# samuel-vitorino/sopro

Measured on AMD Instinct MI355X. Metric: audio_seconds_per_second, higher is better.
Workload: dtype f32; 1 GPU; Sopro-135M synthesize, 32 utterances x 200 frames per GPU (BASELINE configs[1]), S=64 text tokens, 32 distinct 150-frame reference voice(s) per batch prepared outside the timed region, top_p=0.9 T=1.05 anti_loop (reference defaults), synthetic weights with EOS suppressed; batch_per_gpu=32, frames=200, voices_per_batch=32, parallelism=replicas x1 (utterance sharding, no collective), lanes_per_gpu=4

## Files before the change

include/sopro_hip.h:

```cpp
#ifndef SOPRO_HIP_H
#define SOPRO_HIP_H

#include <stdint.h>

#ifdef __cplusplus
extern "C" {
#endif

#define SOPRO_ABI_VERSION 43

const char* sopro_last_error(void);
int sopro_abi_version(void);
int sopro_build_flags(void);
int sopro_set_lds_floor(int bytes);
int sopro_set_host_wait(int blocking);
int sopro_device_info(int device, int* out4);

int sopro_capture_begin(void* stream);
int sopro_capture_end(void* stream, void** graph_exec_out);
int sopro_graph_launch(void* graph_exec, void* stream);
int sopro_graph_launch_n(void* graph_exec, void* stream, int32_t n);
int sopro_graph_destroy(void* graph_exec);
int sopro_stream_create_cu_range(int first_cu, int n_cus, void** stream_out);
int sopro_stream_create_cu_mask(const uint32_t* mask, int32_t words, void** stream_out);
// ... 14 lines not shown
  float* C; int64_t ldc; int64_t c_seg_stride;
  const float* R; int64_t ldr; int64_t r_seg_stride;
  const float* scale;
  const float* pro_vec;
  long long* dbg;
  int32_t M, N, K, rows_per_seg;
  int32_t prologue, epilogue;
} sopro_gemm_args;
int sopro_gemm_f32(const sopro_gemm_args* args, void* stream);
int sopro_gemm_set_tile_override(int cfg);

typedef struct sopro_gemm_split_ext {
  int32_t a_format;
  int32_t c_mode;
  float* C2; int64_t ldc2; int64_t c2_seg_stride;
  int32_t rms_norm; float rms_eps;
  int32_t ksplit;
  int32_t n_tickets;
  float* ws; int64_t ws_bytes;
  int32_t* tickets;
  int32_t group_m;
  float acc_scale;
  int32_t* range_events;
  const float* rope_cos; const float* rope_sin;
  int32_t rope_cols, rope_dh, rope_pos0, rope_rows_per_seg;
  const float* ln_stats;
  float* ln_stats_out;
} sopro_gemm_split_ext;
int sopro_gemm_bf16x3(const sopro_gemm_args* a, const void* packed_w, const sopro_gemm_split_ext* ext, void* stream);
int64_t sopro_packed_w_rows_bytes(int32_t N, int32_t K);
int sopro_pack_w_rows_bf16(const float* W, int64_t ldw, int32_t N, int32_t K, void* packed, void* stream);
int sopro_gemm_8p_takes(const sopro_gemm_args* a, const sopro_gemm_split_ext* ext);
int sopro_gemm_bf16x3_8p(const sopro_gemm_args* a, const void* w_rows, const sopro_gemm_split_ext* ext, void* stream);
int sopro_gemm_bf16x6(const sopro_gemm_args* a, const void* packed_w, const sopro_gemm_split_ext* ext, void* stream);
int sopro_gemm_bf16x1(const sopro_gemm_args* a, const void* packed_w, const sopro_gemm_split_ext* ext, void* stream);
int sopro_pack_w_bf16(const float* W, int64_t ldw, int32_t N, int32_t K, int32_t pieces, void* packed, void* stream);
int sopro_pack_w_f16x2(const float* W, int64_t ldw, int32_t N, int32_t K, float wscale, void* packed, void* stream);
float sopro_f16x3_a_scale(void);
int sopro_gemm_f16x3(const sopro_gemm_args* a, const void* packed_w, const sopro_gemm_split_ext* ext, void* stream);
int64_t sopro_packed_w_bytes(int32_t N, int32_t K, int32_t pieces);
int sopro_gemm_bf16_set_tile_override(int cfg);
int sopro_gemm_set_group_m(int g);
int sopro_gemm_auto_ksplit(int32_t M, int32_t N, int32_t K, int32_t pieces, int32_t f16, int32_t epilogue, int64_t ws_bytes, int32_t n_tickets);

typedef struct sopro_skinny_args {
  const float* X; int64_t ldx;
  const float* W; int64_t ldw;
  const float* bias;
  float* Y; int64_t ldy;
  const float* R; int64_t ldr;
  const float* scale;
  float* ring;
  const float* dw_w;
  const float* dw_b;
  const int32_t* step;
  const float* Xp; int64_t xp_stride;
  int64_t y_part_stride;
  long long* dbg;
  float eps;
  int32_t B, N, K, epilogue;
  int32_t ring_len, ring_bcap, dil, ksize;
  int32_t np, ksplit, rms_norm;
  int32_t w_layout;
  const float* aux_W; const float* aux_bias; const float* aux_R; float* aux_Y;
  int64_t aux_ldy, aux_ldr, aux_y_part_stride;
  int32_t aux_tiles, aux_flags;
  int32_t ring_format;
  int32_t mt, nt;
} sopro_skinny_args;
int sopro_skinny_f32(const sopro_skinny_args* args, void* stream);
int sopro_pack_skinny_w(const float* W, int64_t ldw, int32_t N, int32_t K, int32_t glu, float* out, void* stream);
int64_t sopro_skinny_packed_floats(int32_t N, int32_t K, int32_t glu);
int sopro_pack_skinny_w_bf16(const float* W, int64_t ldw, int32_t N, int32_t K, int32_t glu, void* out, void* stream);

int sopro_fill2d_u32(void* p, int64_t pitch, int32_t rows, int32_t width, uint32_t value, void* stream);
int sopro_copy2d_u32(void* dst, int64_t dpitch, const void* src, int64_t spitch, int32_t rows, int32_t width, void* stream);
int sopro_nar_seed_i32(int32_t* tokens, int32_t Q, const int32_t* cb0, int64_t cb0_bstride, int32_t B, int32_t T, int32_t vmax, void* stream);
int sopro_cvt_f32_bf16(const float* src, void* dst, int64_t n, void* stream);
int sopro_cvt_bf16_f32(const void* src, float* dst, int64_t n, void* stream);
enum { SOPRO_NORM_RMS = 0, SOPRO_NORM_LN = 1 };
int sopro_norm_f32(const float* x, int64_t ldx, int64_t x_seg_stride , float* out, int64_t ldo, const float* w, const float* b,
                   const float* mul, const float* add, int32_t rows, int32_t rows_per_seg, int32_t C,
                   float eps, int32_t kind, void* stream);
int sopro_row_stats_f32(const float* x, int64_t ldx, int64_t x_seg_stride , int32_t rows, int32_t rows_per_seg, int32_t C,
                        float* stats, void* stream);
int sopro_rms_match_f32(const float* a, const float* x, float* out, int32_t rows, int32_t C, void* stream);
int sopro_tanh_affine_f32(const float* in, float* out, float c0, float c1, int64_t n, void* stream);
int sopro_add_pos_f32(const float* rowvec, const float* table, float* out, int32_t B, int32_t T, int32_t C,
                      int32_t pos0, void* stream);
int sopro_masked_mean_f32(const float* x, const int32_t* lens, float* out, int32_t B, int32_t T, int32_t C,
                          void* stream);

int sopro_stats_pool_f32(const float* h, const float* logit, const int32_t* lens, float* out, int32_t B, int32_t T,
                         int32_t C, void* stream);
int sopro_l2norm_f32(const float* x, float* out, int32_t rows, int32_t C, float eps, void* stream);

int sopro_dwconv_f32(const float* x, const float* w, const float* bias, const float* res, float* out,
                     const int32_t* lens, int32_t B, int32_t T, int32_t C, int32_t ksize, int32_t dil,
                     int32_t left, int32_t mode, void* stream);

int sopro_codebook_sum_f32(const int32_t* tok, int32_t ldt, const int32_t* col, const int32_t* off, const float* wq,
                           int32_t nq, const float* table, int64_t table_rows, const float* base, float alpha,
                           float beta, float* out, int64_t ldo, int64_t o_seg_stride, int32_t rows,
                           int32_t rows_per_seg, int32_t D, void* stream);
int sopro_text_embed_f32(const int32_t* ids, const int32_t* lens, const float* table, int64_t table_rows,
                         const float* pe, float* out, int32_t B, int32_t T, int32_t C, void* stream);
int sopro_argmax_rows_f32(const float* x, int64_t ldx, int32_t* out, int64_t ldo, int32_t inner, int32_t rows, int32_t N,
                          void* stream);
int sopro_argmax_partials_i32(const float* partials, int64_t ldp, int32_t* out, int64_t ldo, int32_t heads, int32_t per_head, int32_t V,
                              int32_t rows, void* stream);

int sopro_fir1_f32(const float* x, int64_t x_seg_stride, int32_t n_in, const float* w, const float* bias, float* out,
                   int64_t ldo, int64_t o_seg_stride, int32_t B, int32_t n_out, int32_t C, int32_t K, int32_t stride,
                   int32_t left, void* stream);
int sopro_rvq_assign_f32(const float* scores, int64_t lds, int32_t V, const float* table, float* res, int64_t ldr,
                         int32_t D, int32_t* codes, int64_t ldc, int32_t rows, void* stream);

typedef struct sopro_attn_args {
  const float* Q; int64_t ldq; int64_t q_bstride;
  const float* K; int64_t ldk; int64_t k_bstride;
  const float* V; int64_t ldv; int64_t v_bstride;
  float* O; int64_t ldo; int64_t o_bstride;
  const int32_t* klens;
  int32_t B, H, dh, Tq, Tk;
  int32_t causal, q_pos0, k_pos0, window;
  float scale;
  const int32_t* kv_index;
} sopro_attn_args;
int sopro_attention_f32(const sopro_attn_args* args, void* stream);
int sopro_attention_split_bf16(const sopro_attn_args* args, int32_t passes, void* stream);
int sopro_attn_decode_f32(const sopro_attn_args* args, void* stream);
typedef struct sopro_xattn_args {
  const float* X; int64_t ldx;
  const float* Xp; int64_t xp_stride;
  const float* norm_w;
  const float* Kp; const float* Vp;
  const int32_t* klens;
  float* Y; int64_t y_part_stride;
  float eps, gate, scale;
  int32_t np, B, H, D, S_cap;
  const float* Qp; int64_t qp_stride;
  int32_t nqp, k_unfolded;
  int32_t kv_format;
} sopro_xattn_args;
int sopro_xattn_step_f32(const sopro_xattn_args* args, void* stream);

int sopro_rope_f32(float* x, int64_t ldx, const float* cos_t, const float* sin_t, int32_t rows,
                   int32_t rows_per_seg, int32_t pos0, int32_t H, int32_t dh, void* stream);

int sopro_upsample2_f32(const float* x, const float* w, float* y, int64_t y_seg_stride, int32_t B, int32_t T,
                        int32_t C, void* stream);
int sopro_final_conv_f32(const float* h, int64_t h_seg_stride, const float* w, float bias, float* wav,
                         int64_t wav_seg_stride, int32_t B, int32_t T, void* stream);

int sopro_seanet_tail_f32(const float* h, int64_t h_seg_stride, const float* w1, const float* b1, const float* w2,
                          const float* b2, const float* wf, float bf, float* wav, int64_t wav_seg_stride, int32_t B,
                          int32_t T, void* stream);
int sopro_seanet_tail_p_f32(const float* h, int64_t h_seg_stride, const float* w1, const float* b1, const float* w2,
                            const float* b2, const float* wf, float bf, float* wav, int64_t wav_seg_stride, int32_t B,
                            int32_t T, int32_t passes, void* stream);
int sopro_seanet_res128_f32(const float* h, int64_t h_seg_stride, const float* w1, const float* b1, const float* w2, const float* b2,
                            float* out, int64_t out_seg_stride, int32_t B, int32_t T, void* stream);
int sopro_seanet_res128_p_f32(const float* h, int64_t h_seg_stride, const float* w1, const float* b1, const float* w2, const float* b2,
                              float* out, int64_t out_seg_stride, int32_t B, int32_t T, int32_t passes , void* stream);
int sopro_seanet_res_set_tiles(int tiles);
int sopro_seanet_up128_f32(const float* x, int64_t x_seg_stride, const float* w, const float* bias, float* out,
// ... 325 lines not shown
```

sopro_amd/csrc/common.h:

```cpp
#pragma once
#ifdef SOPRO_DEV_SWITCHES
#define SOPRO_DEV_ENV(name) getenv(name)
#else
#define SOPRO_DEV_ENV(name) (static_cast<const char*>(nullptr))
#endif
#include <hip/hip_runtime.h>
#include <stdint.h>
#include <stdio.h>
#include <string.h>

#include "../../include/sopro_hip.h"

typedef float f32x4 __attribute__((ext_vector_type(4)));
typedef float f32x16 __attribute__((ext_vector_type(16)));

void sopro_set_error(const char* fmt, ...);
extern int g_sopro_lds_floor;

#define SOPRO_CHECK_ARG(cond, msg)                                  \
  do {                                                              \
    if (!(cond)) {                                                  \
      sopro_set_error("%s: bad argument: %s", __func__, msg);       \
      return -2;                                                    \
    }                                                               \
  } while (0)

#define SOPRO_HIP(call)                                                                   \
  do {                                                                                    \
    hipError_t e_ = (call);                                                               \
    if (e_ != hipSuccess) {                                                               \
      sopro_set_error("%s: %s failed: %s", __func__, #call, hipGetErrorString(e_));       \
      return -1;                                                                          \
    }                                                                                     \
  } while (0)

#define SOPRO_LAUNCH_CHECK()                                                              \
  do {                                                                                    \
    hipError_t e_ = hipGetLastError();                                                    \
    if (e_ != hipSuccess) {                                                               \
      sopro_set_error("%s: kernel launch failed: %s", __func__, hipGetErrorString(e_));   \
      return -1;                                                                          \
    }                                                                                     \
    return 0;                                                                             \
  } while (0)

static inline bool aligned16(const void* p) { return (reinterpret_cast<uintptr_t>(p) & 15u) == 0; }

#define SOPRO_SET_MAX_LDS_ONCE(kern, bytes)                                                                              \
  do {                                                                                                                   \
    static unsigned char done_[64] = {};                                                                                 \
    int dev_ = 0;                                                                                                        \
    SOPRO_HIP(hipGetDevice(&dev_));                                                                                      \
    if (!done_[dev_ & 63]) {                                                                                             \
      SOPRO_HIP(hipFuncSetAttribute(reinterpret_cast<const void*>(kern), hipFuncAttributeMaxDynamicSharedMemorySize, (int)(bytes))); \
      done_[dev_ & 63] = 1;                                                                                              \
    }                                                                                                                    \
  } while (0)

__device__ __forceinline__ float gelu_erf(float v) { return v * 0.5f * (1.0f + erff(v * 0.70710678118654752440f)); }
__device__ __forceinline__ float gelu_fast(float v) {
  const float x = fabsf(v) * 0.70710678118654752440f;
  const float t = __builtin_amdgcn_rcpf(fmaf(0.3275911f, x, 1.0f));
  float p = fmaf(1.061405429f, t, -1.453152027f);
  p = fmaf(p, t, 1.421413741f);
  p = fmaf(p, t, -0.284496736f);
  p = fmaf(p, t, 0.254829592f);
  p *= t;
  const float e = __builtin_amdgcn_exp2f(x * x * -1.44269504088896340736f);
  const float y = fmaf(-p, e, 1.0f);
  const float h = 0.5f * v;
  return fmaf(h, copysignf(y, v), h);
}
__device__ __forceinline__ float sigmoidf_(float v) { return 1.0f / (1.0f + expf(-v)); }
__device__ __forceinline__ float sigmoid_fast(float v) { return __builtin_amdgcn_rcpf(1.0f + __builtin_amdgcn_exp2f(-1.44269504088896340736f * v)); }
__device__ __forceinline__ float eluf_(float v) { return __builtin_amdgcn_fmed3f(v, __expf(v) - 1.0f, 0.0f); }

typedef __bf16 bf16x2_t __attribute__((ext_vector_type(2)));
typedef float f32x2_t __attribute__((ext_vector_type(2)));
__device__ __forceinline__ void split2_bf16(float x, float y, unsigned& hi, unsigned& lo) {
  const f32x2_t v = {x, y};
  const bf16x2_t h = __builtin_convertvector(v, bf16x2_t);
  hi = *reinterpret_cast<const unsigned*>(&h);
  const f32x2_t r = {x - __uint_as_float(hi << 16), y - __uint_as_float(hi & 0xffff0000u)};
  const bf16x2_t l = __builtin_convertvector(r, bf16x2_t);
  lo = *reinterpret_cast<const unsigned*>(&l);
}

#ifndef SOPRO_NT_BULK
#define SOPRO_NT_BULK 1
#endif
__device__ __forceinline__ bool bulk_nt(bool big) { return SOPRO_NT_BULK == 1 || (SOPRO_NT_BULK == 2 && big); }
typedef unsigned u32x4_t __attribute__((ext_vector_type(4)));
typedef unsigned u32x2_t __attribute__((ext_vector_type(2)));
__device__ __forceinline__ void bulk_store4(float* p, const float4& v, bool big) {
  if (bulk_nt(big)) __builtin_nontemporal_store((f32x4){v.x, v.y, v.z, v.w}, reinterpret_cast<f32x4*>(p));
  else *reinterpret_cast<float4*>(p) = v;
}
__device__ __forceinline__ void bulk_store1(float* p, float v, bool big) {
  if (bulk_nt(big)) __builtin_nontemporal_store(v, p);
  else *p = v;
}
__device__ __forceinline__ void bulk_store_u2(void* p, const uint2& v, bool big) {
  if (bulk_nt(big)) __builtin_nontemporal_store((u32x2_t){v.x, v.y}, reinterpret_cast<u32x2_t*>(p));
  else *reinterpret_cast<uint2*>(p) = v;
}
__device__ __forceinline__ void bulk_store_u1(void* p, unsigned v, bool big) {
  if (bulk_nt(big)) __builtin_nontemporal_store(v, reinterpret_cast<unsigned*>(p));
  else *reinterpret_cast<unsigned*>(p) = v;
}
__device__ __forceinline__ uint4 bulk_load16(const void* p, bool big) {
  if (bulk_nt(big)) {
    const u32x4_t v = __builtin_nontemporal_load(reinterpret_cast<const u32x4_t*>(p));
    return make_uint4(v.x, v.y, v.z, v.w);
  }
  return *reinterpret_cast<const uint4*>(p);
}
constexpr int64_t SOPRO_BIG_BYTES = (int64_t)64 << 20;

__device__ __forceinline__ int xcd_contiguous(int b, int n) {
  const int per = n >> 3, rem = n & 7;
  const int x = b & 7, i = b >> 3;
  return x * per + min(x, rem) + i;
}

__device__ __forceinline__ float wave_sum(float v) {
#pragma unroll
  for (int o = 32; o > 0; o >>= 1) v += __shfl_xor(v, o, 64);
  return v;
}
__device__ __forceinline__ float wave_max(float v) {
#pragma unroll
  for (int o = 32; o > 0; o >>= 1) v = fmaxf(v, __shfl_xor(v, o, 64));
  return v;
}

__device__ __forceinline__ void wave_lds_sync() {
  __builtin_amdgcn_fence(__ATOMIC_RELEASE, "wavefront");
  __builtin_amdgcn_wave_barrier();
  __builtin_amdgcn_fence(__ATOMIC_ACQUIRE, "wavefront");
}

struct sopro_prof_scope {
  void* rec;
  hipStream_t s;
  sopro_prof_scope(const char* family, double flops, hipStream_t s);
  ~sopro_prof_scope();
  sopro_prof_scope(const sopro_prof_scope&) = delete;
  sopro_prof_scope& operator=(const sopro_prof_scope&) = delete;
};
```

sopro_amd/csrc/elementwise.hip:

```cpp
#include "common.h"

namespace {

constexpr int NORM_MAX_PER_LANE = 16;

__global__ __launch_bounds__(256) void norm_kernel(const float* __restrict__ x, int64_t ldx, int64_t x_seg_stride, float* __restrict__ out,
                                                   int64_t ldo, const float* __restrict__ w, const float* __restrict__ b,
                                                   const float* __restrict__ mul, const float* __restrict__ add, int rows,
                                                   int rows_per_seg, int C, float eps, int kind) {
  const int lane = threadIdx.x & 63;
  const int row = blockIdx.x * 4 + (threadIdx.x >> 6);
  if (row >= rows) return;
  const int seg = row / rows_per_seg;
  const float* xr = x + (int64_t)seg * x_seg_stride + (int64_t)(row - seg * rows_per_seg) * ldx;
  float v[NORM_MAX_PER_LANE];
  const int per = (C + 63) / 64;
  float s = 0.f;
#pragma unroll
  for (int j = 0; j < NORM_MAX_PER_LANE; ++j) {
    const int c = lane + j * 64;
    v[j] = (j < per && c < C) ? xr[c] : 0.f;
    s += v[j];
  }
  float mean = 0.f, var;
  if (kind == SOPRO_NORM_LN) {
    mean = wave_sum(s) / (float)C;
    float q = 0.f;
#pragma unroll
    for (int j = 0; j < NORM_MAX_PER_LANE; ++j) {
      const int c = lane + j * 64;
      const float d = (j < per && c < C) ? v[j] - mean : 0.f;
      q += d * d;
    }
    var = wave_sum(q) / (float)C;
  } else {
    float q = 0.f;
#pragma unroll
    for (int j = 0; j < NORM_MAX_PER_LANE; ++j) q += v[j] * v[j];
    var = wave_sum(q) / (float)C;
  }
  const float rstd = rsqrtf(var + eps);
  const float* mr = mul ? mul + (int64_t)seg * C : nullptr;
  const float* ar = add ? add + (int64_t)seg * C : nullptr;
  float* orow = out + (int64_t)row * ldo;
#pragma unroll
  for (int j = 0; j < NORM_MAX_PER_LANE; ++j) {
    const int c = lane + j * 64;
    if (j < per && c < C) {
      float y = ((v[j] - mean) * rstd) * w[c];
      if (b) y += b[c];
      if (mr) y *= mr[c];
      if (ar) y += ar[c];
      orow[c] = y;
    }
  }
}

__global__ __launch_bounds__(256) void rms_match_kernel(const float* __restrict__ a, const float* __restrict__ x,
                                                        float* __restrict__ out, int rows, int C) {
  const int lane = threadIdx.x & 63;
  const int row = blockIdx.x * 4 + (threadIdx.x >> 6);
  if (row >= rows) return;
  const float* ar = a + (int64_t)row * C;
  const float* xr = x + (int64_t)row * C;
  float sa = 0.f, sx = 0.f;
  for (int c = lane; c < C; c += 64) {
    sa += ar[c] * ar[c];
    sx += xr[c] * xr[c];
  }
  sa = wave_sum(sa);
  sx = wave_sum(sx);
  const float ra = sqrtf(sa / (float)C + 1e-6f), rx = sqrtf(sx / (float)C + 1e-6f);
  const float sc = fminf(fmaxf(rx / ra, 0.f), 10.f);
  for (int c = lane; c < C; c += 64) out[(int64_t)row * C + c] = ar[c] * sc;
}

__global__ void tanh_affine_kernel(const float* __restrict__ in, float* __restrict__ out, float c0, float c1, int64_t n) {
  const int64_t i = (int64_t)blockIdx.x * blockDim.x + threadIdx.x;
  if (i < n) out[i] = c0 + c1 * tanhf(in[i]);
}

__global__ void add_pos_kernel(const float* __restrict__ rowvec, const float* __restrict__ table, float* __restrict__ out,
                               int B, int T, int C, int pos0) {
  const int64_t i = (int64_t)blockIdx.x * blockDim.x + threadIdx.x;
  const int64_t n = (int64_t)B * T * C;
  if (i >= n) return;
  const int c = (int)(i % C);
  const int64_t bt = i / C;
  const int t = (int)(bt % T), b = (int)(bt / T);
  out[i] = rowvec[(int64_t)b * C + c] + table[(int64_t)(pos0 + t) * C + c];
}

__global__ void masked_mean_kernel(const float* __restrict__ x, const int* __restrict__ lens, float* __restrict__ out,
                                   int B, int T, int C) {
  const int b = blockIdx.y;
  const int c = blockIdx.x * blockDim.x + threadIdx.x;
  if (c >= C) return;
  const int len = lens ? min(lens[b], T) : T;
  float s = 0.f;
  for (int t = 0; t < len; ++t) s += x[((int64_t)b * T + t) * C + c];
  out[(int64_t)b * C + c] = s / ((float)len + 1e-6f);
}

__global__ __launch_bounds__(256) void dwconv_kernel(const float* __restrict__ x, const float* __restrict__ w,
                                                     const float* __restrict__ bias, const float* __restrict__ res,
                                                     float* __restrict__ out, const int* __restrict__ lens, int B, int T,
                                                     int C, int ksize, int dil, int left, int mode) {
  const int c4n = C >> 2;
  const int64_t i = (int64_t)blockIdx.x * blockDim.x + threadIdx.x;
  if (i >= (int64_t)B * T * c4n) return;
  const int c4 = (int)(i % c4n);
  const int64_t bt = i / c4n;
  const int t = (int)(bt % T), b = (int)(bt / T);
  const int len = lens ? min(lens[b], T) : T;
  float4 acc = make_float4(0.f, 0.f, 0.f, 0.f);
  for (int j = 0; j < ksize; ++j) {
    const int ts = t - left + j * dil;
    if (ts < 0 || ts >= len) continue;
    const float4 xv = *reinterpret_cast<const float4*>(x + ((int64_t)b * T + ts) * C + c4 * 4);
    const float4 wv = *reinterpret_cast<const float4*>(w + (int64_t)j * C + c4 * 4);
    acc.x += xv.x * wv.x; acc.y += xv.y * wv.y; acc.z += xv.z * wv.z; acc.w += xv.w * wv.w;
  }
  if (bias) {
    const float4 bv = *reinterpret_cast<const float4*>(bias + c4 * 4);
    acc.x += bv.x; acc.y += bv.y; acc.z += bv.z; acc.w += bv.w;
  }
  const int64_t o = ((int64_t)b * T + t) * C + c4 * 4;
  if (mode == 1) {
    const float4 rv = *reinterpret_cast<const float4*>(res + o);
    acc.x += rv.x; acc.y += rv.y; acc.z += rv.z; acc.w += rv.w;
  } else if (mode == 2) {
    acc.x = gelu_erf(acc.x); acc.y = gelu_erf(acc.y); acc.z = gelu_erf(acc.z); acc.w = gelu_erf(acc.w);
  }
  *reinterpret_cast<float4*>(out + o) = acc;
}

template <int KS>
// ... 311 lines not shown
  if (row >= rows) return;
  float s = 0.f;
  for (int c = lane; c < C; c += 64) s += x[(int64_t)row * C + c] * x[(int64_t)row * C + c];
  s = wave_sum(s);
  const float d = fmaxf(sqrtf(s), eps);
  for (int c = lane; c < C; c += 64) out[(int64_t)row * C + c] = x[(int64_t)row * C + c] / d;
}

inline unsigned nblk(int64_t n, int bs) { return (unsigned)((n + bs - 1) / bs); }


__global__ __launch_bounds__(256) void fill2d_kernel(unsigned* __restrict__ p, int64_t pitch, int rows, int width, unsigned v) {
  const int64_t i = (int64_t)blockIdx.x * blockDim.x + threadIdx.x;
  if (i >= (int64_t)rows * width) return;
  p[(i / width) * pitch + (i % width)] = v;
}
__global__ __launch_bounds__(256) void copy2d_kernel(unsigned* __restrict__ d, int64_t dpitch, const unsigned* __restrict__ s, int64_t spitch, int rows,
                                                     int width) {
  const int64_t i = (int64_t)blockIdx.x * blockDim.x + threadIdx.x;
  if (i >= (int64_t)rows * width) return;
  d[(i / width) * dpitch + (i % width)] = s[(i / width) * spitch + (i % width)];
}

__global__ __launch_bounds__(256) void nar_seed_kernel(int* __restrict__ tokens, int Q, const int* __restrict__ cb0, int64_t bstride, int B, int T, int vmax) {
  const int64_t i = (int64_t)blockIdx.x * blockDim.x + threadIdx.x;
  if (i >= (int64_t)B * T) return;
  const int b = (int)(i / T), t = (int)(i - (int64_t)b * T);
  tokens[i * Q] = min(max(cb0[(int64_t)b * bstride + t], 0), vmax);
}

__global__ __launch_bounds__(256) void cvt_f32_bf16_kernel(const float* __restrict__ src, uint2* __restrict__ dst, int64_t n4) {
  const int64_t i = (int64_t)blockIdx.x * blockDim.x + threadIdx.x;
  if (i >= n4) return;
  const float4 v = reinterpret_cast<const float4*>(src)[i];
  unsigned a, b, lo;
  split2_bf16(v.x, v.y, a, lo);
  split2_bf16(v.z, v.w, b, lo);
  dst[i] = make_uint2(a, b);
}
__global__ __launch_bounds__(256) void cvt_bf16_f32_kernel(const uint2* __restrict__ src, float* __restrict__ dst, int64_t n4) {
  const int64_t i = (int64_t)blockIdx.x * blockDim.x + threadIdx.x;
  if (i >= n4) return;
  const uint2 v = src[i];
  reinterpret_cast<float4*>(dst)[i] = make_float4(__uint_as_float(v.x << 16), __uint_as_float(v.x & 0xffff0000u), __uint_as_float(v.y << 16),
                                                  __uint_as_float(v.y & 0xffff0000u));
}

__global__ __launch_bounds__(256) void row_stats_kernel(const float* __restrict__ x, int64_t ldx, int64_t seg_stride, int rows, int rps, int C,
                                                        float* __restrict__ stats) {
  const int per_row = C >> 2;
  const int64_t i = (int64_t)blockIdx.x * blockDim.x + threadIdx.x;
  const int64_t r = i / per_row;
  if (r >= rows) return;
  const int c4 = (int)(i - r * per_row);
  const int64_t seg = r / rps, rr = r - seg * rps;
  const float4 v = *reinterpret_cast<const float4*>(x + seg * seg_stride + rr * ldx + c4 * 4);
  float s = (v.x + v.y) + (v.z + v.w);
  s += __shfl_xor(s, 1, 64); s += __shfl_xor(s, 2, 64); s += __shfl_xor(s, 4, 64); s += __shfl_xor(s, 8, 64);
  const float mu = s * (1.0f / 64.0f);
  const float dx = v.x - mu, dy = v.y - mu, dz = v.z - mu, dw = v.w - mu;
  float q = (dx * dx + dy * dy) + (dz * dz + dw * dw);
  q += __shfl_xor(q, 1, 64); q += __shfl_xor(q, 2, 64); q += __shfl_xor(q, 4, 64); q += __shfl_xor(q, 8, 64);
  if ((c4 & 15) == 0) *reinterpret_cast<float2*>(stats + (r * (C >> 6) + (c4 >> 4)) * 2) = make_float2(mu, q);
}

}

extern "C" {

int sopro_row_stats_f32(const float* x, int64_t ldx, int64_t x_seg_stride, int32_t rows, int32_t rows_per_seg, int32_t C, float* stats, void* stream) {
  SOPRO_CHECK_ARG(x && stats && rows > 0 && rows_per_seg > 0 && C > 0 && (C & 63) == 0, "x, stats non-NULL; rows > 0; C a multiple of 64");
  SOPRO_CHECK_ARG(aligned16(x) && (ldx & 3) == 0 && (x_seg_stride & 3) == 0 && (reinterpret_cast<uintptr_t>(stats) & 7u) == 0, "16-byte aligned rows, 8-byte aligned stats");
  hipLaunchKernelGGL(row_stats_kernel, dim3(nblk((int64_t)rows * (C >> 2), 256)), dim3(256), 0, (hipStream_t)stream, x, ldx,
                     x_seg_stride ? x_seg_stride : (int64_t)rows_per_seg * ldx, rows, rows_per_seg, C, stats);
  SOPRO_LAUNCH_CHECK();
}

int sopro_norm_f32(const float* x, int64_t ldx, int64_t x_seg_stride, float* out, int64_t ldo, const float* w, const float* b,
                   const float* mul, const float* add, int32_t rows, int32_t rows_per_seg, int32_t C, float eps,
                   int32_t kind, void* stream) {
  SOPRO_CHECK_ARG(x && out && w, "x, out, w must be non-NULL");
  SOPRO_CHECK_ARG(rows > 0 && C > 0 && C <= 64 * NORM_MAX_PER_LANE && rows_per_seg > 0, "rows > 0, 0 < C <= 1024");
  SOPRO_CHECK_ARG(kind == SOPRO_NORM_RMS || kind == SOPRO_NORM_LN, "unknown norm kind");
  hipLaunchKernelGGL(norm_kernel, dim3(nblk(rows, 4)), dim3(256), 0, (hipStream_t)stream, x, ldx,
                     x_seg_stride ? x_seg_stride : (int64_t)rows_per_seg * ldx, out, ldo, w, b, mul, add, rows, rows_per_seg, C, eps, kind);
  SOPRO_LAUNCH_CHECK();
}

int sopro_rms_match_f32(const float* a, const float* x, float* out, int32_t rows, int32_t C, void* stream) {
  SOPRO_CHECK_ARG(a && x && out && rows > 0 && C > 0, "bad pointers or sizes");
  hipLaunchKernelGGL(rms_match_kernel, dim3(nblk(rows, 4)), dim3(256), 0, (hipStream_t)stream, a, x, out, rows, C);
  SOPRO_LAUNCH_CHECK();
}

int sopro_tanh_affine_f32(const float* in, float* out, float c0, float c1, int64_t n, void* stream) {
  SOPRO_CHECK_ARG(in && out && n > 0, "bad pointers or sizes");
  hipLaunchKernelGGL(tanh_affine_kernel, dim3(nblk(n, 256)), dim3(256), 0, (hipStream_t)stream, in, out, c0, c1, n);
  SOPRO_LAUNCH_CHECK();
}

int sopro_add_pos_f32(const float* rowvec, const float* table, float* out, int32_t B, int32_t T, int32_t C, int32_t pos0,
                      void* stream) {
  SOPRO_CHECK_ARG(rowvec && table && out && B > 0 && T > 0 && C > 0 && pos0 >= 0, "bad pointers or sizes");
  hipLaunchKernelGGL(add_pos_kernel, dim3(nblk((int64_t)B * T * C, 256)), dim3(256), 0, (hipStream_t)stream, rowvec, table,
                     out, B, T, C, pos0);
  SOPRO_LAUNCH_CHECK();
}

int sopro_masked_mean_f32(const float* x, const int32_t* lens, float* out, int32_t B, int32_t T, int32_t C, void* stream) {
  SOPRO_CHECK_ARG(x && out && B > 0 && T > 0 && C > 0, "bad pointers or sizes");
  hipLaunchKernelGGL(masked_mean_kernel, dim3(nblk(C, 128), B), dim3(128), 0, (hipStream_t)stream, x, lens, out, B, T, C);
  SOPRO_LAUNCH_CHECK();
}

int sopro_dwconv_f32(const float* x, const float* w, const float* bias, const float* res, float* out, const int32_t* lens,
                     int32_t B, int32_t T, int32_t C, int32_t ksize, int32_t dil, int32_t left, int32_t mode, void* stream) {
  SOPRO_CHECK_ARG(x && w && out && B > 0 && T > 0 && C > 0 && (C & 3) == 0, "bad pointers or sizes (C % 4 == 0)");
  SOPRO_CHECK_ARG(ksize >= 1 && dil >= 1 && left >= 0 && mode >= 0 && mode <= 2, "bad conv geometry or mode");
  SOPRO_CHECK_ARG(mode != 1 || res, "mode 1 needs res");
  SOPRO_CHECK_ARG(aligned16(x) && aligned16(w) && aligned16(out), "pointers must be 16-byte aligned");
  SOPRO_CHECK_ARG((!bias || aligned16(bias)) && (!res || aligned16(res)), "bias / res must be 16-byte aligned");
  static const bool comb_off = SOPRO_DEV_ENV("SOPRO_DWCONV_COMB") != nullptr && SOPRO_DEV_ENV("SOPRO_DWCONV_COMB")[0] == '0';
  if (!comb_off && (ksize == 11 || ksize == 7) && (int64_t)B * T >= 1024 && T >= 8 * dil) {
    const int per_r = ((T + dil - 1) / dil + 7) / 8;
    const dim3 grid(nblk((int64_t)B * dil * per_r * (C / 4), 256));
    if (ksize == 11)
      hipLaunchKernelGGL(dwconv_comb_kernel<11>, grid, dim3(256), 0, (hipStream_t)stream, x, w, bias, res, out, lens, B, T, C, dil, left, mode, per_r);
    else
      hipLaunchKernelGGL(dwconv_comb_kernel<7>, grid, dim3(256), 0, (hipStream_t)stream, x, w, bias, res, out, lens, B, T, C, dil, left, mode, per_r);
    SOPRO_LAUNCH_CHECK();
  }
  hipLaunchKernelGGL(dwconv_kernel, dim3(nblk((int64_t)B * T * (C / 4), 256)), dim3(256), 0, (hipStream_t)stream, x, w, bias,
                     res, out, lens, B, T, C, ksize, dil, left, mode);
  SOPRO_LAUNCH_CHECK();
}

int sopro_codebook_sum_f32(const int32_t* tok, int32_t ldt, const int32_t* col, const int32_t* off, const float* wq,
                           int32_t nq, const float* table, int64_t table_rows, const float* base, float alpha, float beta,
                           float* out, int64_t ldo, int64_t o_seg_stride, int32_t rows, int32_t rows_per_seg, int32_t D,
                           void* stream) {
  SOPRO_CHECK_ARG(tok && col && off && wq && table && out, "NULL pointer");
  SOPRO_CHECK_ARG(rows > 0 && rows_per_seg > 0 && nq > 0 && D > 0 && (D & 3) == 0 && table_rows > 0, "bad sizes (D % 4 == 0)");
  SOPRO_CHECK_ARG(aligned16(table) && aligned16(out) && (ldo & 3) == 0 && (o_seg_stride & 3) == 0, "alignment");
  hipLaunchKernelGGL(codebook_sum_kernel, dim3(nblk((int64_t)rows * (D / 4), 256)), dim3(256), 0, (hipStream_t)stream, tok,
                     ldt, col, off, wq, nq, table, table_rows, base, alpha, beta, out, ldo, o_seg_stride, rows, rows_per_seg, D);
  SOPRO_LAUNCH_CHECK();
}

int sopro_text_embed_f32(const int32_t* ids, const int32_t* lens, const float* table, int64_t table_rows, const float* pe,
                         float* out, int32_t B, int32_t T, int32_t C, void* stream) {
  SOPRO_CHECK_ARG(ids && table && pe && out && B > 0 && T > 0 && C > 0 && (C & 3) == 0, "bad pointers or sizes");
  hipLaunchKernelGGL(text_embed_kernel, dim3(nblk((int64_t)B * T * (C / 4), 256)), dim3(256), 0, (hipStream_t)stream, ids, lens,
                     table, table_rows, pe, out, B, T, C);
  SOPRO_LAUNCH_CHECK();
}

int sopro_argmax_rows_f32(const float* x, int64_t ldx, int32_t* out, int64_t ldo, int32_t inner, int32_t rows, int32_t N,
                          void* stream) {
  SOPRO_CHECK_ARG(x && out && rows > 0 && N > 0 && inner > 0, "bad pointers or sizes");
  hipLaunchKernelGGL(argmax_rows_kernel, dim3(nblk(rows, 4)), dim3(256), 0, (hipStream_t)stream, x, ldx, out, ldo, inner, rows, N);
  SOPRO_LAUNCH_CHECK();
}

int sopro_fir1_f32(const float* x, int64_t x_seg_stride, int32_t n_in, const float* w, const float* bias, float* out, int64_t ldo,
                   int64_t o_seg_stride, int32_t B, int32_t n_out, int32_t C, int32_t K, int32_t stride, int32_t left, void* stream) {
  SOPRO_CHECK_ARG(x && w && out, "NULL pointer");
  SOPRO_CHECK_ARG(B > 0 && B <= 65535 && n_in > 0 && n_out > 0 && C > 0 && K > 0 && stride > 0 && left >= 0 && ldo >= C, "bad sizes");
  hipLaunchKernelGGL(fir1_kernel, dim3(nblk((int64_t)n_out * C, 256), B), dim3(256), 0, (hipStream_t)stream, x, x_seg_stride, n_in, w,
// ... 154 lines not shown
```

sopro_amd/csrc/gemm_bf16s.hip:

```cpp
#include "common.h"
#include "gemm_epilogue.h"
#include "gemm_host.h"

namespace {

constexpr int BK = 32;


typedef __bf16 bf16x8 __attribute__((ext_vector_type(8)));
typedef _Float16 f16x8 __attribute__((ext_vector_type(8)));
typedef _Float16 f16x2_t __attribute__((ext_vector_type(2)));

__device__ __forceinline__ bf16x8 as_frag(const uint4& v) { return *reinterpret_cast<const bf16x8*>(&v); }
__device__ __forceinline__ f16x8 as_frag16(const uint4& v) { return *reinterpret_cast<const f16x8*>(&v); }

constexpr float A16_SCALE = 8.0f;

template <int NPL, bool F16 = false>
__device__ __forceinline__ void split_pair(float x, float y, unsigned (&pc)[NPL]) {
#pragma unroll
  for (int p = 0; p < NPL; ++p) {
    const f32x2_t v = {x, y};
    if constexpr (F16) {
      const f16x2_t h = __builtin_convertvector(v, f16x2_t);
      pc[p] = *reinterpret_cast<const unsigned*>(&h);
      x -= (float)h[0];
      y -= (float)h[1];
    } else {
      const bf16x2_t h = __builtin_convertvector(v, bf16x2_t);
      pc[p] = *reinterpret_cast<const unsigned*>(&h);
      x -= __uint_as_float(pc[p] << 16);
      y -= __uint_as_float(pc[p] & 0xffff0000u);
    }
  }
}

template <int NPL, int WM, int WN, int TM, int TN, int EPI, int AMODE, int OUT, bool SK, bool F16 = false>
__global__ __launch_bounds__(WM* WN * 64) void gemm_bf16s_kernel(const sopro_gemm_args g, const uint4* __restrict__ Wp,
                                                                 int ksubs, const sopro_gemm_split_ext ext) {
  constexpr int AROW = NPL * 64 + 16;
  constexpr bool FOLD = F16;
  constexpr int NT = WM * WN * 64;
  constexpr int BM = WM * TM * 32;
  constexpr int BN = WN * TN * 32;
  constexpr int A_F4 = BM * 8 / NT;
  constexpr int RSTEP = NT / 8;
  extern __shared__ float4 smem4[];
  unsigned char* As = reinterpret_cast<unsigned char*>(smem4);

  const int tid = threadIdx.x, lane = tid & 63, wave = tid >> 6;
  const int wm = wave / WN, wn = wave % WN;
  const int ntn = (g.N + BN - 1) / BN;
  const int bid = xcd_contiguous((int)blockIdx.x, (int)gridDim.x);
  int mt = bid / ntn, nt = bid % ntn;
  if (ext.group_m > 1) {
    const int ntm_all = (g.M + BM - 1) / BM;
    const int per = ext.group_m * ntn;
    const int grp = bid / per, rem = bid - grp * per;
    const int first = grp * ext.group_m;
    const int gsz = min(ntm_all - first, ext.group_m);
    mt = first + rem % gsz;
    nt = rem / gsz;
  }
  const int m0 = mt * BM, n0 = nt * BN;
  const int lrow = tid >> 3, lc4 = tid & 7;
  const int rps = g.rows_per_seg;
  long long* dbg = g.dbg ? g.dbg + (int64_t)blockIdx.x * 8 : nullptr;
  if (dbg && tid == 0) dbg[0] = clock64();

  static_assert(AMODE != 5 || NPL == 1, "bf16 rows are a one-pass (bf16 mode) operand form");
  constexpr int AES = AMODE == 5 ? 2 : 4;
  const char* ap[A_F4];
#pragma unroll
  for (int i = 0; i < A_F4; ++i) {
    const int m = min(m0 + lrow + i * RSTEP, g.M - 1);
    const int seg = m / rps;
    const int r = m - seg * rps;
    ap[i] = reinterpret_cast<const char*>(g.A) + ((int64_t)seg * g.a_seg_stride + (int64_t)r * g.lda) * AES;
  }
  const int ntiles = (g.N + 31) >> 5;
  const uint4* bp[TN];
#pragma unroll
  for (int j = 0; j < TN; ++j) {
    const int t = min((n0 >> 5) + wn * TN + j, ntiles - 1);
    bp[j] = Wp + ((int64_t)t * ksubs * NPL) * 64 + lane;
  }
  int boff[TN];
#pragma unroll
  for (int j = 0; j < TN; ++j) {
    const int t = min((n0 >> 5) + wn * TN + j, ntiles - 1);
    boff[j] = (t * ksubs * NPL) * 64 + lane;
  }
  float biasv[TN];
#pragma unroll
  for (int j = 0; j < TN; ++j) {
    const int n = n0 + (wn * TN + j) * 32 + (lane & 31);
    biasv[j] = (g.bias && n < g.N) ? g.bias[n] : 0.f;
  }

  float4 raA[A_F4], raB[A_F4];
  float ssq[A_F4];
  float rsc[A_F4];
  float a16max = 0.f;
#pragma unroll
  for (int i = 0; i < A_F4; ++i) { ssq[i] = 0.f; rsc[i] = A16_SCALE; }
  float sapin[A_F4];
#pragma unroll
  for (int i = 0; i < A_F4; ++i) sapin[i] = A16_SCALE;
  float lmu[A_F4], lrs[A_F4];
  float4 pvA = make_float4(0.f, 0.f, 0.f, 0.f), pvB = pvA;
  const int KT = (g.K + BK - 1) / BK;
  const int klast = g.K - 4;

  auto gload = [&](int kt, float4 (&ra)[A_F4], float4& pv) {
    const int k = min(kt * BK + lc4 * 4, klast);
    if constexpr (AMODE == 5) {
#pragma unroll
      for (int i = 0; i < A_F4; ++i) {
        const uint2 v = *reinterpret_cast<const uint2*>(ap[i] + (int64_t)k * 2);
        ra[i].x = __uint_as_float(v.x);
        ra[i].y = __uint_as_float(v.y);
      }
    } else {
#pragma unroll
      for (int i = 0; i < A_F4; ++i) ra[i] = *reinterpret_cast<const float4*>(ap[i] + (int64_t)k * 4);
    }
    if (AMODE == 3) pv = *reinterpret_cast<const float4*>(g.pro_vec + k);
  };
  auto bload = [&](int kt, uint4 (&rb)[TN][2][NPL]) {
#pragma unroll
    for (int j = 0; j < TN; ++j)
#pragma unroll
      for (int s = 0; s < 2; ++s)
#pragma unroll
        for (int p = 0; p < NPL; ++p) rb[j][s][p] = bp[j][((int64_t)(kt * 2 + s) * NPL + p) * 64];
  };
  auto lstore_piece = [&](int buf, float4 (&ra)[A_F4], const float4& pv, int i, bool fresh, bool first) {
    if constexpr (FOLD) {
      if constexpr (AMODE == 4) asm volatile("" : "+v"(rsc[i]), "+v"(ssq[i]));
      else asm volatile("" : "+v"(sapin[i]));
    }
    if constexpr (AMODE == 5) {
      unsigned char* a = As + buf * BM * AROW + lrow * AROW + lc4 * 8;
      *reinterpret_cast<uint2*>(a + i * RSTEP * AROW) = make_uint2(__float_as_uint(ra[i].x), __float_as_uint(ra[i].y));
    } else if constexpr (AMODE == 2) {
      unsigned char* a = As + buf * BM * AROW + lrow * AROW + lc4 * 16;
      *reinterpret_cast<f32x4*>(a + i * RSTEP * AROW) = (f32x4){ra[i].x, ra[i].y, ra[i].z, ra[i].w};
    } else {
      if constexpr (AMODE == 1) {
        ra[i].x = eluf_(ra[i].x); ra[i].y = eluf_(ra[i].y); ra[i].z = eluf_(ra[i].z); ra[i].w = eluf_(ra[i].w);
      } else if constexpr (AMODE == 3) {
        ra[i].x += pv.x; ra[i].y += pv.y; ra[i].z += pv.z; ra[i].w += pv.w;
      } else if constexpr (AMODE == 6) {
        const f32x2_t r2 = {lrs[i], lrs[i]}, n2 = {lmu[i], lmu[i]};
        const f32x2_t lo2 = (f32x2_t){ra[i].x, ra[i].y} * r2 + n2, hi2 = (f32x2_t){ra[i].z, ra[i].w} * r2 + n2;
        ra[i].x = lo2[0]; ra[i].y = lo2[1]; ra[i].z = hi2[0]; ra[i].w = hi2[1];
      }
      if constexpr (AMODE == 4) {
        if (fresh) ssq[i] = fmaf(ra[i].x, ra[i].x, fmaf(ra[i].y, ra[i].y, fmaf(ra[i].z, ra[i].z, fmaf(ra[i].w, ra[i].w, ssq[i]))));
      }
      unsigned char* a = As + buf * BM * AROW + lrow * AROW + lc4 * 8;
      {
        unsigned c0[NPL], c1[NPL];
        if constexpr (F16) {
          const float F16MAX = 65504.0f;
          if constexpr (AMODE == 4) {
            if (first) {
              float mx = fmaxf(fmaxf(fabsf(ra[i].x), fabsf(ra[i].y)), fmaxf(fabsf(ra[i].z), fabsf(ra[i].w)));
              mx = fmaxf(mx, __shfl_xor(mx, 1, 64));
              mx = fmaxf(mx, __shfl_xor(mx, 2, 64));
              mx = fmaxf(mx, __shfl_xor(mx, 4, 64));
              const int ex = (int)((__float_as_uint(mx) >> 23) & 255u);
              rsc[i] = (ex == 0 || ex == 255) ? A16_SCALE : __uint_as_float((unsigned)min(max(261 - ex, 2), 252) << 23);
            }
          }
          const float sa = AMODE == 4 ? rsc[i] : sapin[i];
          const float vx = ra[i].x * sa, vy = ra[i].y * sa, vz = ra[i].z * sa, vw = ra[i].w * sa;
          a16max = fmaxf(a16max, fmaxf(fmaxf(fabsf(vx), fabsf(vy)), fmaxf(fabsf(vz), fabsf(vw))));
          split_pair<NPL, true>(__builtin_amdgcn_fmed3f(vx, -F16MAX, F16MAX), __builtin_amdgcn_fmed3f(vy, -F16MAX, F16MAX), c0);
          split_pair<NPL, true>(__builtin_amdgcn_fmed3f(vz, -F16MAX, F16MAX), __builtin_amdgcn_fmed3f(vw, -F16MAX, F16MAX), c1);
        } else {
          split_pair<NPL>(ra[i].x, ra[i].y, c0);
          split_pair<NPL>(ra[i].z, ra[i].w, c1);
        }
#pragma unroll
        for (int p = 0; p < NPL; ++p) *reinterpret_cast<uint2*>(a + i * RSTEP * AROW + p * 64) = make_uint2(c0[p], c1[p]);
      }
    }
  };
  auto lstore = [&](int buf, float4 (&ra)[A_F4], const float4& pv, bool fresh = true, bool first = false) {
#pragma unroll
    for (int i = 0; i < A_F4; ++i) lstore_piece(buf, ra, pv, i, fresh, first);
  };

  f32x16 acc[TM][TN];
#pragma unroll
  for (int i = 0; i < TM; ++i)
#pragma unroll
    for (int j = 0; j < TN; ++j)
#pragma unroll
      for (int r = 0; r < 16; ++r) acc[i][j][r] = 0.f;

  const int frow = lane & 31, fg = lane >> 5;
  constexpr int NPAIR = NPL == 1 ? 1 : (NPL == 2 ? 3 : 6);
  constexpr int PA[6] = {NPL == 1 ? 0 : (NPL == 2 ? 1 : 2), 0, NPL == 2 ? 0 : 1, 1, 0, 0};
  constexpr int PB[6] = {0, NPL == 2 ? 1 : 2, NPL == 2 ? 0 : 1, 0, 1, 0};
  auto compute = [&](int buf, const uint4 (&rb)[TN][2][NPL]) {
    const unsigned char* a = As + buf * BM * AROW + (wm * TM * 32 + frow) * AROW + fg * 16;
#pragma unroll
    for (int s = 0; s < 2; ++s) {
      uint4 af[TM][NPL];
#pragma unroll
      for (int i = 0; i < TM; ++i)
#pragma unroll
        for (int p = 0; p < NPL; ++p) af[i][p] = *reinterpret_cast<const uint4*>(a + i * 32 * AROW + p * 64 + s * 32);
#pragma unroll
      for (int q = 0; q < NPAIR; ++q)
#pragma unroll
        for (int i = 0; i < TM; ++i)
#pragma unroll
          for (int j = 0; j < TN; ++j)
            if constexpr (F16)
              acc[i][j] = __builtin_amdgcn_mfma_f32_32x32x16_f16(as_frag16(af[i][PA[q]]), as_frag16(rb[j][s][PB[q]]), acc[i][j], 0, 0, 0);
// ... 41 lines not shown
          for (int j = 0; j < TN; ++j) {
            if constexpr (F16)
              acc[i][j] = __builtin_amdgcn_mfma_f32_32x32x16_f16(as_frag16(af[i][PA[q]]), as_frag16(rb[j][s][PB[q]]), acc[i][j], 0, 0, 0);
            else
              acc[i][j] = __builtin_amdgcn_mfma_f32_32x32x16_bf16(as_frag(af[i][PA[q]]), as_frag(rb[j][s][PB[q]]), acc[i][j], 0, 0, 0);
            ++m;
            if constexpr (FOLD) {
#pragma unroll
              for (int i = 0; i < A_F4; ++i)
                if (m == NM / 2 + i * (NM / 2) / A_F4) {
                  __builtin_amdgcn_sched_barrier(0x104);
                  lstore_piece(buf ^ 1, rs, pvs, i, fresh_s, false);
                }
            }
            if (m % STRIDE == 0 && nl < NL) {
              if constexpr (NPL == 1) {
                __builtin_amdgcn_sched_barrier(0);
                issue(nl++);
                __builtin_amdgcn_sched_barrier(0);
              } else {
                __builtin_amdgcn_sched_barrier(0x786);
                issue(nl++);
                __builtin_amdgcn_sched_barrier(0x786);
              }
            }
          }
    }
#pragma unroll
    for (int n = 0; n < NL; ++n)
      if (n >= nl) issue(n);
  };

  const int KS = SK ? ext.ksplit : 1;
  const int per = (KT + KS - 1) / KS;
  const int kt0 = (int)blockIdx.y * per;
  const int nkt = max(0, min(KT, kt0 + per) - kt0);
  const int ktl = max(kt0, kt0 + nkt - 1);

  uint4 rb0[TN][2][NPL], rb1[TN][2][NPL];
  constexpr bool DEEP = true;
  gload(min(kt0, KT - 1), raA, pvA);
  bload(min(kt0, KT - 1), rb0);
  if (DEEP) gload(min(min(kt0 + 1, ktl), KT - 1), raB, pvB);
  if constexpr (AMODE == 6) {
    const int P = g.K >> 6;
#pragma unroll
    for (int i = 0; i < A_F4; ++i) {
      const float2* st = reinterpret_cast<const float2*>(ext.ln_stats) + (int64_t)min(m0 + lrow + i * RSTEP, g.M - 1) * P;
      float sm = 0.f;
      for (int p = lc4; p < P; p += 8) sm += st[p].x;
      sm += __shfl_xor(sm, 1, 64); sm += __shfl_xor(sm, 2, 64); sm += __shfl_xor(sm, 4, 64);
      const float mean = sm / (float)P;
      float m2 = 0.f;
      for (int p = lc4; p < P; p += 8) {
        const float2 v = st[p];
        const float d = v.x - mean;
        m2 += fmaf(64.0f * d, d, v.y);
      }
      m2 += __shfl_xor(m2, 1, 64); m2 += __shfl_xor(m2, 2, 64); m2 += __shfl_xor(m2, 4, 64);
      lrs[i] = rsqrtf(m2 / (float)g.K + ext.rms_eps);
      lmu[i] = -mean * lrs[i];
    }
  }
  lstore(0, raA, pvA, true, true);
  __syncthreads();
  if (dbg && tid == 0) dbg[1] = clock64();
  {
    int it = 0;
    for (; it + 1 < nkt; it += 2) {
      const int k1 = min(kt0 + it + 1, ktl), k2 = min(kt0 + it + 2, ktl), k3 = min(kt0 + it + 3, ktl);
      compute_spread(0, rb0, k2, raA, pvA, k1, rb1, raB, pvB, true);
      if constexpr (!FOLD) lstore(1, raB, pvB, true);
      __syncthreads();
      compute_spread(1, rb1, k3, raB, pvB, k2, rb0, raA, pvA, it + 2 < nkt);
      if constexpr (!FOLD) lstore(0, raA, pvA, it + 2 < nkt);
      __syncthreads();
    }
    if (it < nkt) {
      compute(0, rb0);
      __syncthreads();
    }
  }
  if (dbg && tid == 0) dbg[2] = clock64();
  if constexpr (SK) {
    constexpr int PER_THREAD = TM * TN * 16;
    const int tile = bid, ntile = gridDim.x;
    float* mine = ext.ws + ((int64_t)((int64_t)blockIdx.y * ntile + tile) * NT + tid) * PER_THREAD;
#pragma unroll
    for (int i = 0; i < TM; ++i)
#pragma unroll
      for (int j = 0; j < TN; ++j)
#pragma unroll
        for (int r = 0; r < 16; r += 4)
          *reinterpret_cast<float4*>(mine + (i * TN + j) * 16 + r) = make_float4(acc[i][j][r], acc[i][j][r + 1], acc[i][j][r + 2], acc[i][j][r + 3]);
    __syncthreads();
    int* flag = reinterpret_cast<int*>(smem4);
    if (tid == 0) {
      __atomic_thread_fence(__ATOMIC_RELEASE);
      const int old = __hip_atomic_fetch_add(ext.tickets + tile, 1, __ATOMIC_ACQ_REL, __HIP_MEMORY_SCOPE_AGENT);
      *flag = old;
      if (old == KS - 1) __hip_atomic_store(ext.tickets + tile, 0, __ATOMIC_RELAXED, __HIP_MEMORY_SCOPE_AGENT);
    }
    __syncthreads();
    if (*flag != KS - 1) return;
    __atomic_thread_fence(__ATOMIC_ACQUIRE);
    __syncthreads();
#pragma unroll
    for (int i = 0; i < TM; ++i)
#pragma unroll
      for (int j = 0; j < TN; ++j)
#pragma unroll
        for (int r = 0; r < 16; ++r) acc[i][j][r] = 0.f;
    const int64_t sl_stride = (int64_t)ntile * NT * PER_THREAD;
    const float* part0 = ext.ws + ((int64_t)tile * NT + tid) * PER_THREAD;
    for (int s0 = 0; s0 < KS; s0 += 16) {
#pragma unroll
      for (int i = 0; i < TM; ++i)
#pragma unroll
        for (int j = 0; j < TN; ++j)
#pragma unroll
          for (int r = 0; r < 16; r += 4) {
            f32x4 v[16];
#pragma unroll
            for (int u = 0; u < 16; ++u) {
              const int sl = min(s0 + u, KS - 1);
              v[u] = __builtin_nontemporal_load(reinterpret_cast<const f32x4*>(part0 + sl * sl_stride + (i * TN + j) * 16 + r));
            }
#pragma unroll
            for (int u = 0; u < 16; ++u) {
              if (s0 + u < KS) {
                acc[i][j][r] += v[u][0]; acc[i][j][r + 1] += v[u][1]; acc[i][j][r + 2] += v[u][2]; acc[i][j][r + 3] += v[u][3];
              }
            }
          }
    }
  }
  float cscale = 1.0f;
  if constexpr (F16) {
    cscale = AMODE == 4 ? ext.acc_scale * A16_SCALE : ext.acc_scale;
    if (ext.range_events && !(a16max <= 65504.0f)) atomicAdd(ext.range_events, 1);
  }
  const float* rs = nullptr;
  if constexpr (AMODE == 4) {
    float* rsl = reinterpret_cast<float*>(smem4) + BM * (BN + 4);
#pragma unroll
    for (int i = 0; i < A_F4; ++i) {
      float v = ssq[i];
      v += __shfl_xor(v, 1, 64);
      v += __shfl_xor(v, 2, 64);
      v += __shfl_xor(v, 4, 64);
      float r = rsqrtf(v / (float)g.K + ext.rms_eps);
      if constexpr (F16) r *= __uint_as_float(0x7f000000u - __float_as_uint(rsc[i])) * cscale;
      if (lc4 == 0) rsl[lrow + i * RSTEP] = r;
    }
    __syncthreads();
    rs = rsl;
  }
  gemm_store_tile<WM, WN, TM, TN, EPI, OUT>(g, reinterpret_cast<float*>(smem4), acc, biasv, m0, n0, &ext, rs, cscale);
  if (dbg && tid == 0) dbg[3] = clock64();
}

template <int NPL, bool F16 = false>
__global__ __launch_bounds__(256) void pack_w_kernel(const float* __restrict__ W, int64_t ldw, int N, int K, uint4* __restrict__ out,
                                                     int ksubs, int64_t total, float wscale = 1.0f) {
  const int64_t i = (int64_t)blockIdx.x * blockDim.x + threadIdx.x;
  if (i >= total) return;
  const int lane = (int)(i & 63);
  const int64_t pk = i >> 6;
  const int p = (int)(pk % NPL);
  const int64_t tk = pk / NPL;
  const int ks = (int)(tk % ksubs);
  const int t = (int)(tk / ksubs);
  const int n = t * 32 + (lane & 31);
  const int k0 = ks * 16 + (lane >> 5) * 8;
  unsigned w[4];
#pragma unroll
  for (int e = 0; e < 4; ++e) {
    const int k = k0 + 2 * e;
    const float x = (n < N && k < K) ? W[(int64_t)n * ldw + k] : 0.f;
    const float y = (n < N && k + 1 < K) ? W[(int64_t)n * ldw + k + 1] : 0.f;
    unsigned pc[NPL];
    if constexpr (F16) split_pair<NPL, true>(x * wscale, y * wscale, pc);
    else split_pair<NPL>(x, y, pc);
    w[e] = pc[p];
  }
  out[i] = make_uint4(w[0], w[1], w[2], w[3]);
}

template <int NPL, int WM, int WN, int TM, int TN, int EPI, int AMODE, int OUT, bool F16 = false>
int launch_one(const sopro_gemm_args& g, const uint4* wp, int ksubs, const sopro_gemm_split_ext& ext, hipStream_t s) {
  constexpr int BM = WM * TM * 32, BN = WN * TN * 32;
  constexpr size_t lds_main = (size_t)2 * BM * (NPL * 64 + 16), lds_epi = (size_t)BM * (BN + 4 + (AMODE == 4 ? 1 : 0)) * sizeof(float);
  constexpr size_t lds = lds_main > lds_epi ? lds_main : lds_epi;
  const int ks = ext.ksplit > 1 ? ext.ksplit : 1;
  auto kern = ks > 1 ? gemm_bf16s_kernel<NPL, WM, WN, TM, TN, EPI, AMODE, OUT, true, F16> : gemm_bf16s_kernel<NPL, WM, WN, TM, TN, EPI, AMODE, OUT, false, F16>;
  constexpr size_t lds_cap = lds > (size_t)96 * 1024 ? lds : (size_t)96 * 1024;
  if (ks > 1) SOPRO_SET_MAX_LDS_ONCE(kern, lds_cap);
  else SOPRO_SET_MAX_LDS_ONCE(kern, lds_cap);
  const size_t lds_req = lds > (size_t)g_sopro_lds_floor ? lds : (size_t)g_sopro_lds_floor;
  const int ntm = (g.M + BM - 1) / BM, ntn = (g.N + BN - 1) / BN;
  if (ks > 1) {
    const int64_t need = (int64_t)ks * ntm * ntn * BM * BN * (int64_t)sizeof(float);
    if (!ext.ws || !ext.tickets || ext.ws_bytes < need || ext.n_tickets < ntm * ntn) {
      sopro_set_error("split-K needs a %lld-byte workspace and %d tickets (got %lld, %d)", (long long)need, ntm * ntn,
                      (long long)ext.ws_bytes, ext.n_tickets);
      return -2;
    }
  }
  hipLaunchKernelGGL(kern, dim3(ntm * ntn, ks), dim3(WM * WN * 64), lds_req, s, g, wp, ksubs, ext);
  SOPRO_LAUNCH_CHECK();
}

inline int amode_of(const sopro_gemm_args& g, const sopro_gemm_split_ext& ext) {
  if (ext.a_format == 1) return 2;
  if (ext.a_format == 2) return 5;
  if (ext.rms_norm) return 4;
  if (ext.ln_stats) return 6;
  return g.prologue == SOPRO_PRO_ELU ? 1 : (g.prologue == SOPRO_PRO_ADDVEC ? 3 : 0);
}

template <int NPL, int WM, int WN, int TM, int TN>
int launch_cfg3(const sopro_gemm_args& g, const uint4* wp, int ksubs, const sopro_gemm_split_ext& ext, hipStream_t s) {
  const int key = g.epilogue * 100 + amode_of(g, ext) * 10 + ext.c_mode;
#define SOPRO_CASE(E, A, O) \
  case (E) * 100 + (A) * 10 + (O): return launch_one<NPL, WM, WN, TM, TN, ((E) == SOPRO_EPI_GELU ? SOPRO_EPI_GELU_FAST : (E)), A, O>(g, wp, ksubs, ext, s)
  switch (key) {
    SOPRO_CASE(SOPRO_EPI_NONE, 0, 0);
    SOPRO_CASE(SOPRO_EPI_GELU, 0, 0);
    SOPRO_CASE(SOPRO_EPI_RES, 0, 0);
    SOPRO_CASE(SOPRO_EPI_ROPE, 0, 0);
    SOPRO_CASE(SOPRO_EPI_NONE, 6, 0);
    SOPRO_CASE(SOPRO_EPI_GELU, 6, 0);
    SOPRO_CASE(SOPRO_EPI_ROPE, 6, 0);
    SOPRO_CASE(SOPRO_EPI_NONE, 1, 0);
    SOPRO_CASE(SOPRO_EPI_RES, 1, 0);
    SOPRO_CASE(SOPRO_EPI_NONE, 0, 3);
    SOPRO_CASE(SOPRO_EPI_NONE, 0, 4);
    SOPRO_CASE(SOPRO_EPI_RES, 0, 3);
    default: break;
  }
  if constexpr (NPL == 1) {
    switch (key) {
      SOPRO_CASE(SOPRO_EPI_NONE, 0, 7);
      SOPRO_CASE(SOPRO_EPI_NONE, 5, 8);
      SOPRO_CASE(SOPRO_EPI_NONE, 5, 7);
      SOPRO_CASE(SOPRO_EPI_RES, 5, 7);
      SOPRO_CASE(SOPRO_EPI_NONE, 5, 6);
      SOPRO_CASE(SOPRO_EPI_NONE, 5, 0);
      default: break;
    }
  }
  if constexpr (NPL == 2) {
    switch (key) {
      SOPRO_CASE(SOPRO_EPI_NONE, 0, 1);
      SOPRO_CASE(SOPRO_EPI_NONE, 0, 2);
      SOPRO_CASE(SOPRO_EPI_NONE, 2, 0);
      SOPRO_CASE(SOPRO_EPI_NONE, 2, 1);
      SOPRO_CASE(SOPRO_EPI_NONE, 2, 2);
      SOPRO_CASE(SOPRO_EPI_NONE, 2, 4);
      SOPRO_CASE(SOPRO_EPI_RES, 2, 1);
      default: break;
    }
  }
#undef SOPRO_CASE
  sopro_set_error("sopro_gemm_bf16x%d: (epilogue %d, prologue %d, a_format %d, c_mode %d) is not an available combination",
                  NPL == 2 ? 3 : NPL, g.epilogue, g.prologue, ext.a_format, ext.c_mode);
  return -2;
}

template <int NPL, int WM, int WN, int TM, int TN, bool F16 = false>
int launch_cfg6(const sopro_gemm_args& g, const uint4* wp, int ksubs, const sopro_gemm_split_ext& ext, hipStream_t s) {
  const int key = g.epilogue * 10 + amode_of(g, ext);
#define SOPRO_CASE(E, A) \
  case (E) * 10 + (A): return launch_one<NPL, WM, WN, TM, TN, (((E) == SOPRO_EPI_GELU && (F16 || NPL != 3)) ? SOPRO_EPI_GELU_FAST : (E)), A, 0, F16>(g, wp, ksubs, ext, s)
  switch (key) {
    SOPRO_CASE(SOPRO_EPI_NONE, 0);
    SOPRO_CASE(SOPRO_EPI_GELU, 0);
    SOPRO_CASE(SOPRO_EPI_RES, 0);
    SOPRO_CASE(SOPRO_EPI_NONE, 3);
    SOPRO_CASE(SOPRO_EPI_GELU, 4);
    SOPRO_CASE(SOPRO_EPI_NONE, 4);
    default: break;
  }
#undef SOPRO_CASE
  if constexpr (WN * TN * 32 >= 64) {
    constexpr int GLU_ = (F16 || NPL != 3) ? SOPRO_EPI_GLU_FAST : SOPRO_EPI_GLU;
    if (key == SOPRO_EPI_GLU * 10) return launch_one<NPL, WM, WN, TM, TN, GLU_, 0, 0, F16>(g, wp, ksubs, ext, s);
    if (key == SOPRO_EPI_GLU * 10 + 4) return launch_one<NPL, WM, WN, TM, TN, GLU_, 4, 0, F16>(g, wp, ksubs, ext, s);
  }
  sopro_set_error("sopro_gemm_%s: (epilogue %d, prologue %d) is not an available combination", F16 ? "f16x3" : (NPL == 3 ? "bf16x6" : "bf16x1"), g.epilogue, g.prologue);
  return -2;
}

#define SOPRO_TILES(X) \
  X(T64, 2, 2, 1, 1) X(T64x128, 2, 2, 1, 2) X(T128x64, 2, 2, 2, 1) X(T128, 2, 2, 2, 2) X(T256x128, 2, 2, 4, 2) X(T128_W8, 2, 4, 2, 1) X(T128_W1x4, 1, 4, 4, 1)
#define SOPRO_TILE(T, WM, WN, TM, TN) T,
enum Tile { SOPRO_TILES(SOPRO_TILE) };
#undef SOPRO_TILE
struct TileSize { int bm, bn; };
TileSize tile_size(Tile t) {
#define SOPRO_TILE(T, WM, WN, TM, TN) if (t == T) return {WM * TM * 32, WN * TN * 32};
  SOPRO_TILES(SOPRO_TILE)
#undef SOPRO_TILE
  return {0, 0};
}

enum Family { BF16X1, BF16X3, BF16X6, F16X3 };

Tile default_tile(Family f, int M, int N, int epilogue) {
  const Tile small = epilogue == SOPRO_EPI_GLU ? T64x128 : T64;
  switch (f) {
    case BF16X3:
      return (N <= 64 || M <= 64) ? T64 : T128;
    case BF16X1: {
      const int64_t t128 = (int64_t)((M + 127) / 128) * ((N + 127) / 128);
      return (N <= 64 || M <= 64 || t128 < 256) ? small : T128;
    }
    case BF16X6:
      return small;
    case F16X3:
      return M >= 8192 ? T128 : small;
  }
  return T64;
}

enum Form { FORM_CFG3, FORM_CFG6, FORM_ARGMAX };

template <int NPL, bool F16, Form FORM>
constexpr bool has_tile(Tile t) {
#ifdef SOPRO_DEV_SWITCHES
  if (t == T128_W1x4) return NPL == 2 && FORM == (F16 ? FORM_CFG6 : FORM_CFG3);
#endif
  if (t == T64 || t == T128) return true;
  if (FORM != FORM_CFG3) return t == (FORM == FORM_ARGMAX ? T128x64 : T64x128);
  return NPL == 2 && (t == T128x64 || t == T256x128 || t == T128_W8);
}

struct Call {
  sopro_gemm_args g;
  sopro_gemm_split_ext ext;
  const uint4* wp;
  int ksubs;
  hipStream_t s;
};

template <int NPL, bool F16, Form FORM>
int launch_tile(Tile t, const Call& c) {
  switch (t) {
#define SOPRO_TILE(T, WM, WN, TM, TN)                                                                                                     \
  case T:                                                                                                                                 \
    if constexpr (!has_tile<NPL, F16, FORM>(T)) break;                                                                                    \
    else if constexpr (FORM == FORM_ARGMAX) return launch_one<NPL, WM, WN, TM, TN, SOPRO_EPI_NONE, 0, 5, F16>(c.g, c.wp, c.ksubs, c.ext, c.s); \
    else if constexpr (FORM == FORM_CFG6) return launch_cfg6<NPL, WM, WN, TM, TN, F16>(c.g, c.wp, c.ksubs, c.ext, c.s);                  \
    else return launch_cfg3<NPL, WM, WN, TM, TN>(c.g, c.wp, c.ksubs, c.ext, c.s);
    SOPRO_TILES(SOPRO_TILE)
#undef SOPRO_TILE
  }
  sopro_set_error("tile %d is not built for this kernel family", (int)t);
  return -2;
}

template <int NPL, bool F16 = false>
int launch_argmax(const Call& c) {
  const sopro_gemm_args& g = c.g;
  const sopro_gemm_split_ext& ext = c.ext;
  SOPRO_CHECK_ARG(g.epilogue == SOPRO_EPI_NONE && g.prologue == SOPRO_PRO_NONE && !ext.rms_norm && ext.a_format == 0,
                  "arg-max output takes a plain contraction (no prologue / epilogue / fused norm)");
  SOPRO_CHECK_ARG(ext.C2 && ext.ldc2 >= (g.N + 63) / 64, "arg-max output: C2 = [M][ldc2 >= ceil(N / 64)] (value, index) pairs");
  static const bool tm1 = SOPRO_DEV_ENV("SOPRO_ARGMAX_TM") != nullptr && SOPRO_DEV_ENV("SOPRO_ARGMAX_TM")[0] == '1';
  static const bool tn1 = SOPRO_DEV_ENV("SOPRO_ARGMAX_TN") != nullptr && SOPRO_DEV_ENV("SOPRO_ARGMAX_TN")[0] == '1';
  Tile t = T64;
  if (g.M >= 8192 && !tm1) t = (g.N >= 2048 && (g.N & 127) == 0 && !tn1) ? T128 : T128x64;
  return launch_tile<NPL, F16, FORM_ARGMAX>(t, c);
}

int check_rope(const sopro_gemm_args& g, const sopro_gemm_split_ext& ext) {
  if (g.epilogue != SOPRO_EPI_ROPE) return 0;
  const int dh = ext.rope_dh;
  SOPRO_CHECK_ARG(ext.rope_cos && ext.rope_sin && aligned16(ext.rope_cos) && aligned16(ext.rope_sin), "EPI_ROPE needs 16-byte aligned cos / sin tables");
  SOPRO_CHECK_ARG(dh >= 8 && dh <= 64 && (dh & (dh - 1)) == 0, "EPI_ROPE: rope_dh must be a power of two in 8..64 (heads must not straddle a 64-column tile)");
  SOPRO_CHECK_ARG(ext.rope_cols > 0 && ext.rope_cols <= g.N && ext.rope_cols % dh == 0, "EPI_ROPE: rope_cols must be whole heads within N");
  SOPRO_CHECK_ARG(ext.rope_rows_per_seg > 0 && ext.rope_pos0 >= 0, "EPI_ROPE: rope_rows_per_seg > 0, rope_pos0 >= 0");
  SOPRO_CHECK_ARG(ext.c_mode == 0 && ext.a_format == 0 && g.prologue == SOPRO_PRO_NONE && !ext.rms_norm, "EPI_ROPE is a plain fp32-rows form");
  SOPRO_CHECK_ARG((g.N & 3) == 0 && (g.ldc & 3) == 0 && (g.c_seg_stride & 3) == 0 && aligned16(g.C), "EPI_ROPE: 16-byte aligned output rows");
  return 0;
}

int check_ln(const sopro_gemm_args& g, const sopro_gemm_split_ext& ext) {
  if (ext.ln_stats) {
    SOPRO_CHECK_ARG((g.K & 63) == 0 && (reinterpret_cast<uintptr_t>(ext.ln_stats) & 7u) == 0, "fused LayerNorm: K % 64 == 0, 8-byte aligned ln_stats");
    SOPRO_CHECK_ARG(ext.a_format == 0 && g.prologue == SOPRO_PRO_NONE && !ext.rms_norm && ext.c_mode == 0, "fused LayerNorm takes plain fp32 rows (no prologue, c_mode 0)");
    SOPRO_CHECK_ARG(g.epilogue == SOPRO_EPI_NONE || g.epilogue == SOPRO_EPI_GELU || g.epilogue == SOPRO_EPI_ROPE, "fused LayerNorm: epilogue NONE, GELU or ROPE");
    SOPRO_CHECK_ARG(ext.rms_eps > 0.f, "fused LayerNorm: rms_eps carries the norm's eps (> 0)");
  }
  if (ext.ln_stats_out) {
    SOPRO_CHECK_ARG(g.epilogue == SOPRO_EPI_RES && ext.c_mode == 0 && (g.N & 63) == 0 && (reinterpret_cast<uintptr_t>(ext.ln_stats_out) & 7u) == 0,
                    "ln_stats_out: an EPI_RES contraction with fp32 output rows, N % 64 == 0, 8-byte aligned pairs");
    SOPRO_CHECK_ARG((g.ldc & 3) == 0 && (g.c_seg_stride & 3) == 0 && aligned16(g.C) && (g.ldr & 3) == 0 && (g.r_seg_stride & 3) == 0 && aligned16(g.R),
                    "ln_stats_out: 16-byte aligned output / residual rows");
  }
  return 0;
}

int check_common(sopro_gemm_args& g, sopro_gemm_split_ext& ext, const void* packed_w) {
  if (int rc = gemm_check_basic(__func__, g, &ext, packed_w, GEMM_PACKED_W)) return rc;
  SOPRO_CHECK_ARG(ext.ksplit >= 0 && ext.ksplit <= 64, "ksplit must be in 0..64");
  SOPRO_CHECK_ARG(ext.ksplit <= 1 || g.dbg == nullptr, "the clock-stamp probe is for unsplit launches");
  return 0;
}

int check_rms(const char* who, const sopro_gemm_args& g, const sopro_gemm_split_ext& ext, bool plain_out) {
  SOPRO_CHECK_AS(who, !ext.rms_norm || ((g.K & 31) == 0 && ext.ksplit <= 1 && g.prologue == SOPRO_PRO_NONE && ext.rms_eps > 0.f && (!plain_out || ext.c_mode == 0)),
                 plain_out ? "fused RMSNorm needs K % 32 == 0, no split-K, no prologue, eps > 0 and a plain output"
                           : "fused RMSNorm needs K % 32 == 0, no split-K, no prologue and eps > 0");
  return 0;
}

int g_group_m = 0;

typedef int (*forms_check)(const char* who, const sopro_gemm_args& g, const sopro_gemm_split_ext& ext);
int prepare(const char* who, const sopro_gemm_args* a, const void* packed_w, const sopro_gemm_split_ext* x, void* stream, bool ext_required,
            forms_check forms, Call& c) {
  SOPRO_CHECK_AS(who, a != nullptr && (x != nullptr || !ext_required), ext_required ? "args / ext is NULL (ext carries acc_scale)" : "args is NULL");
  c.g = *a;
  memset(&c.ext, 0, sizeof(c.ext));
  if (x) c.ext = *x;
  if (c.ext.group_m == 0) c.ext.group_m = g_group_m;
  if (forms)
    if (int rc = forms(who, c.g, c.ext)) return rc;
  if (int rc = check_common(c.g, c.ext, packed_w)) return rc;
  if (int rc = check_ln(c.g, c.ext)) return rc;
  c.wp = reinterpret_cast<const uint4*>(packed_w);
  c.ksubs = (c.g.K + 31) / 32 * 2;
  c.s = reinterpret_cast<hipStream_t>(stream);
  return 0;
}

int forms_bf16x1(const char* who, const sopro_gemm_args& g, const sopro_gemm_split_ext& ext) {
  SOPRO_CHECK_AS(who, (ext.a_format == 0 || ext.a_format == 2) && (ext.c_mode == 0 || (ext.c_mode >= 3 && ext.c_mode <= 8)),
                 "bf16x1 reads fp32 rows (a_format 0) or bf16 rows (2) and writes fp32 rows (c_mode 0, 3, 4), arg-max partials (5) or bf16 rows (6, 7, 8)");
  if (ext.a_format == 2 || ext.c_mode >= 6) {
    SOPRO_CHECK_AS(who, !ext.rms_norm && g.prologue == SOPRO_PRO_NONE && (g.epilogue == SOPRO_EPI_NONE || g.epilogue == SOPRO_EPI_RES),
                   "bf16 rows: no prologue / fused norm, epilogue NONE or RES (the activation is applied by the producer: c_mode 7 / 8)");
    SOPRO_CHECK_AS(who, ext.a_format != 2 || ((g.lda & 3) == 0 && (g.a_seg_stride & 3) == 0), "bf16 A rows: lda, a_seg_stride multiples of 4 elements");
    SOPRO_CHECK_AS(who, g.epilogue != SOPRO_EPI_RES || ext.c_mode >= 6, "EPI_RES with bf16 A writes bf16 rows (its skip operand R is bf16 then)");
  }
  return check_rms(who, g, ext, true);
}

template <bool F16>
int forms_x6(const char* who, const sopro_gemm_args& g, const sopro_gemm_split_ext& ext) {
  if (F16) SOPRO_CHECK_AS(who, ext.acc_scale > 0.f, "acc_scale = 1 / (sopro_f16x3_a_scale() * the weight's pack scale) must be set");
  SOPRO_CHECK_AS(who, ext.a_format == 0 && (ext.c_mode == 0 || ext.c_mode == 5),
                 F16 ? "the f16 three-pass path reads fp32 rows and writes fp32 rows, or arg-max partials (c_mode 5)"
                     : "the six-pass path reads fp32 rows and writes fp32 rows, or arg-max partials (c_mode 5)");
  return check_rms(who, g, ext, false);
}

}

extern "C" int sopro_gemm_set_group_m(int g) {
  g_group_m = g > 1 ? g : 0;
  return 0;
}

static bool eight_waves(const sopro_gemm_args& g) {
  static const bool on = SOPRO_DEV_ENV("SOPRO_GEMM_W8") != nullptr && SOPRO_DEV_ENV("SOPRO_GEMM_W8")[0] == '1';
  return on && g.N >= 512 && g.M >= 1024;
}

#ifdef SOPRO_DEV_SWITCHES
bool sopro_gemm_astat_takes(const sopro_gemm_args& g, const sopro_gemm_split_ext& ext);
int sopro_gemm_astat_bf16x3(const sopro_gemm_args& g, const void* packed_w, hipStream_t s);
#endif

static int g_tile_override = 0;
extern "C" int sopro_gemm_bf16_set_tile_override(int cfg) {
  g_tile_override = cfg;
  return 0;
}

extern "C" int sopro_gemm_auto_ksplit(int32_t M, int32_t N, int32_t K, int32_t pieces, int32_t f16, int32_t epilogue, int64_t ws_bytes, int32_t n_tickets) {
  static const bool no_splitk = getenv("SOPRO_NO_SPLITK") && getenv("SOPRO_NO_SPLITK")[0] == '1';
  if (no_splitk || M <= 0 || N <= 0 || K <= 0) return 1;
  if (f16 && M >= 8192) return 1;
  const TileSize t = tile_size(default_tile(f16 ? F16X3 : pieces == 3 ? BF16X6 : pieces == 1 ? BF16X1 : BF16X3, M, N, epilogue));
  const int64_t tiles = (int64_t)((M + t.bm - 1) / t.bm) * ((N + t.bn - 1) / t.bn);
  const int kt = (K + 31) / 32;
  if (tiles >= 96 || kt < 32 || tiles > n_tickets) return 1;
  int ks = (int)lrint(sqrt(2.5 * kt));
  if (ks > 16) ks = 16;
  if (ks > 512 / (int)tiles) ks = 512 / (int)tiles;
  if (ks < 1) ks = 1;
  while (ks > 1 && (int64_t)ks * tiles * t.bm * t.bn * 4 > ws_bytes) --ks;
  return ks;
}

extern "C" int64_t sopro_packed_w_bytes(int32_t N, int32_t K, int32_t pieces) {
  if (N <= 0 || K <= 0 || pieces < 1 || pieces > 3) return 0;
  return (int64_t)((N + 31) / 32) * ((K + 31) / 32 * 2) * pieces * 64 * 16;
}

extern "C" int sopro_pack_w_bf16(const float* W, int64_t ldw, int32_t N, int32_t K, int32_t pieces, void* packed, void* stream) {
  SOPRO_CHECK_ARG(W && packed && N > 0 && K > 0 && ldw >= K, "bad pointers or sizes");
  SOPRO_CHECK_ARG(pieces >= 1 && pieces <= 3, "pieces must be 1 (bf16x1), 2 (bf16x3) or 3 (bf16x6)");
  SOPRO_CHECK_ARG(aligned16(packed), "packed must be 16-byte aligned");
  const int ksubs = (K + 31) / 32 * 2;
  const int64_t total = (int64_t)((N + 31) / 32) * ksubs * pieces * 64;
  const dim3 grid((unsigned)((total + 255) / 256));
  if (pieces == 1)
    hipLaunchKernelGGL(pack_w_kernel<1>, grid, dim3(256), 0, (hipStream_t)stream, W, ldw, N, K, reinterpret_cast<uint4*>(packed), ksubs, total);
  else if (pieces == 2)
    hipLaunchKernelGGL(pack_w_kernel<2>, grid, dim3(256), 0, (hipStream_t)stream, W, ldw, N, K, reinterpret_cast<uint4*>(packed), ksubs, total);
  else
    hipLaunchKernelGGL(pack_w_kernel<3>, grid, dim3(256), 0, (hipStream_t)stream, W, ldw, N, K, reinterpret_cast<uint4*>(packed), ksubs, total);
  SOPRO_LAUNCH_CHECK();
}

extern "C" int sopro_gemm_bf16x3(const sopro_gemm_args* a, const void* packed_w, const sopro_gemm_split_ext* x, void* stream) {
  Call c;
  if (int rc = prepare(__func__, a, packed_w, x, stream, false, nullptr, c)) return rc;
  const sopro_gemm_args& g = c.g;
  const sopro_gemm_split_ext& ext = c.ext;
  SOPRO_CHECK_ARG(g.prologue == SOPRO_PRO_NONE || g.prologue == SOPRO_PRO_ELU, "prologue must be NONE or ELU");
  SOPRO_CHECK_ARG(g.epilogue == SOPRO_EPI_NONE || g.epilogue == SOPRO_EPI_GELU || g.epilogue == SOPRO_EPI_RES || g.epilogue == SOPRO_EPI_ROPE,
                  "epilogue must be NONE, GELU, RES or ROPE");
  if (int rc = check_rope(g, ext)) return rc;
  SOPRO_CHECK_ARG(ext.a_format == 0 || ext.a_format == 1, "a_format must be 0 (fp32) or 1 (split form)");
  SOPRO_CHECK_ARG(!ext.rms_norm, "fused RMSNorm is a six-pass (sopro_gemm_bf16x6) feature");
  if (ext.a_format == 1) {
    SOPRO_CHECK_ARG(g.prologue == SOPRO_PRO_NONE, "split-form A carries its activation already");
    SOPRO_CHECK_ARG((g.K & 31) == 0 && (g.lda & 31) == 0 && (g.a_seg_stride & 31) == 0 && (reinterpret_cast<uintptr_t>(g.A) & 127u) == 0,
                    "split-form A: K, lda, a_seg_stride multiples of 32 and a 128-byte aligned base");
  }
  SOPRO_CHECK_ARG(ext.c_mode >= 0 && ext.c_mode <= 4, "c_mode must be 0..4");
  if (int rc = gemm_check_out_rows(__func__, g, ext, true)) return rc;
#ifdef SOPRO_DEV_SWITCHES
  if (g_tile_override == 9 && sopro_gemm_astat_takes(g, ext)) return sopro_gemm_astat_bf16x3(g, packed_w, c.s);
// ... 83 lines not shown
```

sopro_amd/csrc/gemm_epilogue.h:

```cpp
#pragma once
#include "common.h"

constexpr int SOPRO_EPI_GELU_FAST = 100;
constexpr int SOPRO_EPI_GLU_FAST = 101;
template <int WM, int WN, int TM, int TN, int EPI, int OUT = 0>
__device__ __forceinline__ void gemm_store_tile(const sopro_gemm_args& g, float* __restrict__ Cs, f32x16 (&acc)[TM][TN],
                                                const float (&biasv)[TN], int m0, int n0,
                                                const sopro_gemm_split_ext* __restrict__ ext = nullptr,
                                                const float* __restrict__ rs = nullptr, float cscale = 1.0f) {
  constexpr int NT = WM * WN * 64;
  constexpr int BM = WM * TM * 32;
  constexpr int BN = WN * TN * 32;
  const int tid = threadIdx.x, lane = tid & 63, wave = tid >> 6;
  const int wm = wave / WN, wn = wave % WN;
  const int rps = g.rows_per_seg;
  const bool big = (int64_t)g.M * g.N * (OUT >= 6 ? 2 : 4) >= SOPRO_BIG_BYTES;
  constexpr int CLD = BN + 4;
  constexpr bool RES_AHEAD = EPI == SOPRO_EPI_RES && OUT < 5;
  constexpr int RA_TPR = BN / 4, RA_RPP = NT / RA_TPR, RA_NPASS = BM / RA_RPP;
  float4 rahead[RES_AHEAD ? RA_NPASS : 1];
  const bool whole_tile = m0 + BM <= g.M && n0 + BN <= g.N && (m0 / rps) == ((m0 + BM - 1) / rps);
  if constexpr (RES_AHEAD) {
    const int prow = tid / RA_TPR, ocol = n0 + (tid % RA_TPR) * 4;
    const bool rvec = ((g.N & 3) == 0) && ((g.ldr & 3) == 0) && ((g.r_seg_stride & 3) == 0) && ((reinterpret_cast<uintptr_t>(g.R) & 15u) == 0);
    int m = m0 + prow;
    int seg = m / rps, rr = m - seg * rps;
    if (whole_tile && rvec) {
      const float* rptr = g.R + (int64_t)seg * g.r_seg_stride + (int64_t)rr * g.ldr + ocol;
      const int64_t rstep = (int64_t)RA_RPP * g.ldr;
#pragma unroll
      for (int q = 0; q < RA_NPASS; ++q) rahead[q] = *reinterpret_cast<const float4*>(rptr + q * rstep);
    } else {
#pragma unroll
    for (int q = 0; q < RA_NPASS; ++q) {
      rahead[q] = make_float4(0.f, 0.f, 0.f, 0.f);
      if (ocol < g.N && m < g.M) {
        const float* rptr = g.R + (int64_t)seg * g.r_seg_stride + (int64_t)rr * g.ldr + ocol;
        if (rvec) {
          rahead[q] = *reinterpret_cast<const float4*>(rptr);
        } else {
          rahead[q].x = rptr[0];
          if (ocol + 1 < g.N) rahead[q].y = rptr[1];
          if (ocol + 2 < g.N) rahead[q].z = rptr[2];
          if (ocol + 3 < g.N) rahead[q].w = rptr[3];
        }
      }
      m += RA_RPP; rr += RA_RPP;
      while (rr >= rps) { rr -= rps; ++seg; }
    }
    }
  }
  {
    const int col = lane & 31;
#pragma unroll
    for (int i = 0; i < TM; ++i)
#pragma unroll
      for (int k = 0; k < 4; ++k) {
        const int row0 = (wm * TM + i) * 32 + 8 * k + 4 * (lane >> 5);
        float rs4[4] = {cscale, cscale, cscale, cscale};
        if (rs) {
          const float4 t = *reinterpret_cast<const float4*>(rs + row0);
          rs4[0] = t.x; rs4[1] = t.y; rs4[2] = t.z; rs4[3] = t.w;
        }
#pragma unroll
        for (int j = 0; j < TN; ++j)
#pragma unroll
          for (int e = 0; e < 4; ++e) {
            float p = acc[i][j][4 * k + e] * rs4[e];
            if (rs) asm("" : "+v"(p));
            Cs[(row0 + e) * CLD + (wn * TN + j) * 32 + col] = p + biasv[j];
          }
      }
  }
  __syncthreads();
#ifdef SOPRO_DEV_SWITCHES
  if (g.dbg && tid == 0) g.dbg[(int64_t)blockIdx.x * 8 + 4] = clock64();
#endif
  if constexpr (OUT == 5) {
    constexpr int TPR5 = NT / BM;
    constexpr int CPT = BN / TPR5;
    const int row = tid / TPR5, part = tid % TPR5;
    float best = -INFINITY;
    int bi = 0x7fffffff;
#pragma unroll 8
    for (int c = 0; c < CPT; ++c) {
      const int n = n0 + part * CPT + c;
      const float v = Cs[row * CLD + part * CPT + c];
      if (n < g.N && v > best) { best = v; bi = n; }
    }
    constexpr int GRP = CPT >= 64 ? 1 : 64 / CPT;
    static_assert(BN % 64 == 0 && (CPT >= 64 ? CPT == 64 : 64 % CPT == 0), "arg-max partials are per 64 columns");
#pragma unroll
    for (int o = 1; o < GRP; o <<= 1) {
      const float ov = __shfl_xor(best, o, 64);
      const int oi = __shfl_xor(bi, o, 64);
      if (ov > best || (ov == best && oi < bi)) { best = ov; bi = oi; }
    }
    if (part % GRP == 0 && m0 + row < g.M) {
      float* pp = ext->C2 + ((int64_t)(m0 + row) * ext->ldc2 + n0 / 64 + part / GRP) * 2;
      pp[0] = best;
      pp[1] = __int_as_float(bi);
    }
    return;
  }
  if constexpr (OUT >= 6) {
    constexpr bool hres = EPI == SOPRO_EPI_RES;
    static_assert(EPI == SOPRO_EPI_NONE || EPI == SOPRO_EPI_RES, "bf16 rows take EPI_NONE or EPI_RES");
    constexpr int HTPR = BN / 4, HRPP = NT / HTPR, HNPASS = BM / HRPP;
    const int prow = tid / HTPR, pc4 = tid % HTPR;
    const int ocol = n0 + pc4 * 4;
    const bool col_ok = ocol < g.N;
    float4 sc4 = make_float4(1.f, 1.f, 1.f, 1.f);
    if (hres && g.scale && col_ok) sc4 = make_float4(g.scale[ocol], g.scale[ocol + 1], g.scale[ocol + 2], g.scale[ocol + 3]);
    int m = m0 + prow;
    int seg = m / rps, rr = m - seg * rps;
    char* const rawb = reinterpret_cast<char*>(g.C);
    char* const actb = OUT == 8 ? reinterpret_cast<char*>(ext->C2) : rawb;
    const int64_t ldact = OUT == 8 ? ext->ldc2 : g.ldc, segact = OUT == 8 ? ext->c2_seg_stride : g.c_seg_stride;
    const char* const rb = reinterpret_cast<const char*>(g.R);
    auto at = [&](int64_t sg, int64_t r, int64_t ld, int64_t sstride) { return (sg * sstride + r * ld + ocol) * 2; };
    const float* csrc = Cs + prow * CLD + pc4 * 4;
    constexpr int HB = HNPASS < 8 ? HNPASS : 8;
#pragma unroll 1
    for (int p0 = 0; p0 < HNPASS; p0 += HB) {
      int64_t oraw[HB], oact[HB];
      bool okq[HB];
      uint2 rv[HB];
#pragma unroll
      for (int q = 0; q < HB; ++q) {
        okq[q] = col_ok && m < g.M;
        oraw[q] = at(seg, rr, g.ldc, g.c_seg_stride);
        oact[q] = at(seg, rr, ldact, segact);
        rv[q] = make_uint2(0u, 0u);
        if (hres && okq[q]) rv[q] = *reinterpret_cast<const uint2*>(rb + at(seg, rr, g.ldr, g.r_seg_stride));
        m += HRPP; rr += HRPP;
        while (rr >= rps) { rr -= rps; ++seg; }
      }
#pragma unroll
      for (int q = 0; q < HB; ++q) {
        if (!okq[q]) continue;
        float4 v = *reinterpret_cast<const float4*>(csrc + (p0 + q) * HRPP * CLD);
        if (hres) {
          v.x = __uint_as_float(rv[q].x << 16) + sc4.x * v.x; v.y = __uint_as_float(rv[q].x & 0xffff0000u) + sc4.y * v.y;
          v.z = __uint_as_float(rv[q].y << 16) + sc4.z * v.z; v.w = __uint_as_float(rv[q].y & 0xffff0000u) + sc4.w * v.w;
        }
        unsigned lo_;
        if (OUT != 7) {
          uint2 h;
          split2_bf16(v.x, v.y, h.x, lo_);
          split2_bf16(v.z, v.w, h.y, lo_);
          bulk_store_u2(rawb + oraw[q], h, big);
        }
        if (OUT != 6) {
          uint2 h;
          split2_bf16(eluf_(v.x), eluf_(v.y), h.x, lo_);
          split2_bf16(eluf_(v.z), eluf_(v.w), h.y, lo_);
          bulk_store_u2(actb + oact[q], h, big);
        }
      }
    }
    return;
  }
  constexpr bool glu = EPI == SOPRO_EPI_GLU || EPI == SOPRO_EPI_GLU_FAST;
  constexpr bool res = EPI == SOPRO_EPI_RES;
  if constexpr (glu && OUT == 0) {
    constexpr int GT = BN / 4, GRPP = NT / GT, GNP = BM / GRPP;
    const int prow = tid / GT, t = tid % GT;
    const int grp = t >> 4, u = t & 15;
    const int ocol = ((n0 + grp * 64) >> 6) * 32 + 2 * u;
    const bool col_ok = n0 + grp * 64 < g.N;
    const bool st2 = ((g.ldc & 1) == 0) && ((g.c_seg_stride & 1) == 0) && ((reinterpret_cast<uintptr_t>(g.C) & 7u) == 0);
    const float* csrc = Cs + prow * CLD + grp * 64 + 2 * u;
    auto piece = [&](int q, float* cp) {
      const float2 v = *reinterpret_cast<const float2*>(csrc + q * GRPP * CLD), gt = *reinterpret_cast<const float2*>(csrc + q * GRPP * CLD + 32);
      const float ox = v.x * (EPI == SOPRO_EPI_GLU_FAST ? sigmoid_fast(gt.x) : sigmoidf_(gt.x)), oy = v.y * (EPI == SOPRO_EPI_GLU_FAST ? sigmoid_fast(gt.y) : sigmoidf_(gt.y));
      if (st2) {
        bulk_store_u2(cp, make_uint2(__float_as_uint(ox), __float_as_uint(oy)), big);
      } else {
        cp[0] = ox;
        cp[1] = oy;
      }
    };
    if (!col_ok) return;
    if (m0 + BM <= g.M && (m0 / rps) == ((m0 + BM - 1) / rps)) {
      const int m = m0 + prow, seg = m / rps, rr = m - seg * rps;
      float* cptr = g.C + (int64_t)seg * g.c_seg_stride + (int64_t)rr * g.ldc + ocol;
      const int64_t cstep = (int64_t)GRPP * g.ldc;
#pragma unroll
      for (int q = 0; q < GNP; ++q) {
        piece(q, cptr + q * cstep);
#ifdef SOPRO_DEV_SWITCHES
        if (g.dbg && tid == 0 && q == GNP / 2 - 1) g.dbg[(int64_t)blockIdx.x * 8 + 5] = clock64();
#endif
      }
    } else {
#pragma unroll 1
      for (int q = 0; q < GNP; ++q) {
        const int m = m0 + prow + q * GRPP;
        if (m >= g.M) break;
        const int seg = m / rps, rr = m - seg * rps;
        piece(q, g.C + (int64_t)seg * g.c_seg_stride + (int64_t)rr * g.ldc + ocol);
      }
    }
    return;
  }
  constexpr int TPR = BN / 4;
  constexpr int RPP = NT / TPR;
  constexpr int NPASS = BM / RPP;
  const int prow = tid / TPR, pc4 = tid % TPR;
  const int n_out_total = glu ? g.N / 2 : g.N;
  const int ncol = n0 + pc4 * 4;
  const int ocol = glu ? (ncol >> 6) * 32 + (ncol & 31) : ncol;
  const bool col_ok = ocol < n_out_total && (!glu || ((pc4 * 4) & 32) == 0);
  const bool vec_ok = ((n_out_total & 3) == 0) && ((g.ldc & 3) == 0) && ((g.c_seg_stride & 3) == 0) &&
                      ((reinterpret_cast<uintptr_t>(g.C) & 15u) == 0) &&
                      (!res || (((g.ldr & 3) == 0) && ((g.r_seg_stride & 3) == 0) && ((reinterpret_cast<uintptr_t>(g.R) & 15u) == 0)));
  float4 sc4 = make_float4(1.f, 1.f, 1.f, 1.f);
  if (res && g.scale) {
    sc4.x = ncol + 0 < g.N ? g.scale[ncol + 0] : 1.f; sc4.y = ncol + 1 < g.N ? g.scale[ncol + 1] : 1.f;
    sc4.z = ncol + 2 < g.N ? g.scale[ncol + 2] : 1.f; sc4.w = ncol + 3 < g.N ? g.scale[ncol + 3] : 1.f;
  }
  int m = m0 + prow;
  int seg = m / rps, rr = m - seg * rps;
  float* cptr = g.C + (int64_t)seg * g.c_seg_stride + (int64_t)rr * g.ldc + ocol;
  constexpr bool second = OUT == 2 || OUT == 4;
  constexpr bool split_out = OUT == 1 || OUT == 2;
  float* const dbase = second ? ext->C2 : g.C;
  const int64_t ldd = second ? ext->ldc2 : g.ldc, dseg = second ? ext->c2_seg_stride : g.c_seg_stride;
  const int64_t dcol_bytes = split_out ? (int64_t)(ocol >> 5) * 128 + (ocol & 31) * 2 : (int64_t)ocol * 4;
  char* dptr = OUT != 0 ? reinterpret_cast<char*>(dbase + (int64_t)seg * dseg + (int64_t)rr * ldd) + dcol_bytes : nullptr;
  const int64_t dstep = (int64_t)RPP * ldd * 4;
  const int64_t cstep = (int64_t)RPP * g.ldc;
  const float* csrc = Cs + prow * CLD + pc4 * 4;
  constexpr int BATCH = NPASS < 8 ? NPASS : 8;
  static_assert(!RES_AHEAD || (RA_NPASS == NPASS && RA_RPP == RPP), "the residual pieces requested ahead are the store loop's");
  auto emit = [&](int pq, float* cpq, char* dpq, const float4& rvq) {
    {
      float4 v = *reinterpret_cast<const float4*>(csrc + pq * RPP * CLD);
      if (glu) {
        const float4 gt = *reinterpret_cast<const float4*>(csrc + pq * RPP * CLD + 32);
        v.x *= sigmoidf_(gt.x); v.y *= sigmoidf_(gt.y); v.z *= sigmoidf_(gt.z); v.w *= sigmoidf_(gt.w);
      } else if (EPI == SOPRO_EPI_GELU) {
        v.x = gelu_erf(v.x); v.y = gelu_erf(v.y); v.z = gelu_erf(v.z); v.w = gelu_erf(v.w);
      } else if (EPI == SOPRO_EPI_GELU_FAST) {
        v.x = gelu_fast(v.x); v.y = gelu_fast(v.y); v.z = gelu_fast(v.z); v.w = gelu_fast(v.w);
      } else if (EPI == SOPRO_EPI_TANH) {
        v.x = tanhf(v.x); v.y = tanhf(v.y); v.z = tanhf(v.z); v.w = tanhf(v.w);
      } else if (res) {
        v.x = rvq.x + sc4.x * v.x; v.y = rvq.y + sc4.y * v.y; v.z = rvq.z + sc4.z * v.z; v.w = rvq.w + sc4.w * v.w;
        if (OUT == 0 && ext && ext->ln_stats_out) {
          float s1 = (v.x + v.y) + (v.z + v.w);
          s1 += __shfl_xor(s1, 1, 64); s1 += __shfl_xor(s1, 2, 64); s1 += __shfl_xor(s1, 4, 64); s1 += __shfl_xor(s1, 8, 64);
          const float mu = s1 * (1.0f / 64.0f);
          const float dx = v.x - mu, dy = v.y - mu, dz = v.z - mu, dw = v.w - mu;
          float s2 = (dx * dx + dy * dy) + (dz * dz + dw * dw);
          s2 += __shfl_xor(s2, 1, 64); s2 += __shfl_xor(s2, 2, 64); s2 += __shfl_xor(s2, 4, 64); s2 += __shfl_xor(s2, 8, 64);
          if ((pc4 & 15) == 0) {
            const int64_t mq = m0 + prow + pq * RPP;
            *reinterpret_cast<float2*>(ext->ln_stats_out + (mq * (g.N >> 6) + (ncol >> 6)) * 2) = make_float2(mu, s2);
          }
        }
      } else if (EPI == SOPRO_EPI_ROPE) {
        if (ncol < ext->rope_cols) {
          const int half = ext->rope_dh >> 1, e = ncol & (ext->rope_dh - 1);
          const bool lowh = e < half;
          const float4 pv = *reinterpret_cast<const float4*>(csrc + pq * RPP * CLD + (lowh ? half : -half));
          const int mq = m0 + prow + pq * RPP;
          const int64_t ti = (int64_t)(ext->rope_pos0 + mq % ext->rope_rows_per_seg) * half + (e & (half - 1));
          const float4 c4 = *reinterpret_cast<const float4*>(ext->rope_cos + ti), s4 = *reinterpret_cast<const float4*>(ext->rope_sin + ti);
          if (lowh) { v.x = v.x * c4.x - pv.x * s4.x; v.y = v.y * c4.y - pv.y * s4.y; v.z = v.z * c4.z - pv.z * s4.z; v.w = v.w * c4.w - pv.w * s4.w; }
          else { v.x = v.x * c4.x + pv.x * s4.x; v.y = v.y * c4.y + pv.y * s4.y; v.z = v.z * c4.z + pv.z * s4.z; v.w = v.w * c4.w + pv.w * s4.w; }
        }
      }
      if (split_out) {
        uint2 h, l;
        split2_bf16(eluf_(v.x), eluf_(v.y), h.x, l.x);
        split2_bf16(eluf_(v.z), eluf_(v.w), h.y, l.y);
        *reinterpret_cast<uint2*>(dpq) = h;
        *reinterpret_cast<uint2*>(dpq + 64) = l;
        if (OUT == 1) return;
      } else if (OUT != 0) {
        bulk_store4(reinterpret_cast<float*>(dpq), make_float4(eluf_(v.x), eluf_(v.y), eluf_(v.z), eluf_(v.w)), big);
        if (OUT == 3) return;
      }
      if (vec_ok) {
        bulk_store4(cpq, v, big);
      } else {
        cpq[0] = v.x;
        if (ocol + 1 < n_out_total) cpq[1] = v.y;
        if (ocol + 2 < n_out_total) cpq[2] = v.z;
        if (ocol + 3 < n_out_total) cpq[3] = v.w;
      }
    }
  };
  if (whole_tile && vec_ok) {
    if (col_ok) {
#pragma unroll
      for (int q = 0; q < NPASS; ++q) {
        emit(q, cptr + q * cstep, OUT != 0 ? dptr + q * dstep : nullptr, rahead[RES_AHEAD ? q : 0]);
#ifdef SOPRO_DEV_SWITCHES
        if (g.dbg && tid == 0 && q == BATCH - 1) g.dbg[(int64_t)blockIdx.x * 8 + 5] = clock64();
#endif
      }
    }
    return;
  }
  auto batch = [&](int p0, const float4* rvb) {
    float* cp[BATCH];
    char* dp[BATCH];
    float4 rv[BATCH];
#pragma unroll
    for (int q = 0; q < BATCH; ++q) {
      const bool ok = col_ok && m < g.M;
      cp[q] = ok ? cptr : nullptr;
      dp[q] = dptr;
      rv[q] = res ? rvb[q] : make_float4(0.f, 0.f, 0.f, 0.f);
      m += RPP; rr += RPP; cptr += cstep;
      if (OUT != 0) dptr += dstep;
      if (rr >= rps) {
        do { rr -= rps; ++seg; } while (rr >= rps);
        cptr = g.C + (int64_t)seg * g.c_seg_stride + (int64_t)rr * g.ldc + ocol;
        if (OUT != 0) dptr = reinterpret_cast<char*>(dbase + (int64_t)seg * dseg + (int64_t)rr * ldd) + dcol_bytes;
      }
    }
#pragma unroll
    for (int q = 0; q < BATCH; ++q) {
      if (!cp[q]) continue;
      emit(p0 + q, cp[q], dp[q], rv[q]);
    }
  };
  if constexpr (RES_AHEAD) {
#pragma unroll
    for (int b = 0; b < NPASS / BATCH; ++b) {
      batch(b * BATCH, rahead + b * BATCH);
#ifdef SOPRO_DEV_SWITCHES
      if (g.dbg && tid == 0 && b == 0) g.dbg[(int64_t)blockIdx.x * 8 + 5] = clock64();
#endif
    }
  } else {
#pragma unroll 1
    for (int p0 = 0; p0 < NPASS; p0 += BATCH) {
      batch(p0, nullptr);
#ifdef SOPRO_DEV_SWITCHES
      if (g.dbg && tid == 0 && p0 == 0) g.dbg[(int64_t)blockIdx.x * 8 + 5] = clock64();
#endif
    }
  }
}
```

sopro_amd/csrc/stages.hip:

```cpp
#include <stdlib.h>

#include <algorithm>
#include <map>
#include <string>
#include <vector>

#include "common.h"

int sopro_stream_batch_append(float* cur, float* other, const float* qkv, int32_t hs, int32_t rows, int64_t bstride, int32_t n, int32_t kv_len,
                              int32_t nkeep, hipStream_t s);
int sopro_stream_batch_gather(float* kv, const int32_t* keep, int32_t n_keep, int32_t layers, int32_t rows_cap, int64_t bstride, int32_t hs, int32_t half,
                              int32_t kv_len, hipStream_t s);
int sopro_spk_frames_launch(const int32_t* tok, int64_t row_stride, int32_t Q, const int32_t* col, const int32_t* off, const float* cw, const float* emb,
                            int64_t table_rows, int32_t SD, const float* w0, const float* b0, const float* w3, const float* b3, const float* W1,
                            const float* b1, const float* w2, const float* b2, const int32_t* lens, int32_t rows, int32_t t_cap, float* h_ws,
                            float* lg_ws, float* dbg_h, float* dbg_lg, hipStream_t s);
int sopro_spk_pool_launch(const float* h_ws, const float* lg_ws, const int32_t* lens, int32_t rows, int32_t t_cap, int32_t SD, const float* Wp,
                          const float* bp, int32_t svd, float* sv, int64_t sv_stride, hipStream_t s);

namespace {

struct Ten {
  const void* p = nullptr;
  int64_t shape[4] = {0, 0, 0, 0};
// ... 899 lines not shown
                           vdst, B, S, p.S_cap, D, H, RMS_EPS, s));
    if (c.precision == 1) {
      STG(sopro_cvt_f32_bf16(kdst, p.kp[i], (int64_t)B * H * p.S_cap * D, s));
      STG(sopro_cvt_f32_bf16(vdst, p.vp[i], (int64_t)B * H * p.S_cap * D, s));
    }
  }
  for (int i = 0; i < c.n_layers_ar; ++i) {
    const int64_t n = (int64_t)((c.ar_kernel - 1) * c.ar_dilations[i] + 1) * B * D;
    STG(sopro_fill2d_u32(p.rings[i], n, 1, (int32_t)n, 0u, s));
  }
  STG(sopro_fill2d_u32(p.hist, (int64_t)B * Tar, 1, B * Tar, 0u, s));
  for (int k = 0; k < 8; ++k) {
    uint32_t u;
    memcpy(&u, &params[k], 4);
    STG(sopro_fill2d_u32(p.params + k, 1, 1, 1, u, s));
  }
  STG(sopro_fill2d_u32(p.nonce, B, 1, B, nonce, s));
  STG(sopro_fill2d_u32(p.key, 1, 1, 1, (uint32_t)seed, s));
  STG(sopro_fill2d_u32(p.key + 1, 1, 1, 1, (uint32_t)(seed >> 32), s));
  sopro_ar_state& st = p.st;
  memset(&st, 0, sizeof(st));
  st.x_cur = p.x[0]; st.cond = p.cond; st.emb = F(e, "cb_embed"); st.hist = p.hist;
  st.step = p.ctr; st.row_step = p.row_step; st.n_stopped = p.ctr + 2;
  st.first_eos = p.first_eos; st.stop_t = p.stop_t; st.recent = p.recent; st.params = p.params; st.nonce = p.nonce;
  st.key = p.key; st.seed = 0; st.B = B; st.D = D; st.Tar = Tar; st.max_steps = Tar; st.V = c.codebook_size; st.bos_row = c.bos_row;
  STG(sopro_ar_init(&st, s));
  if (p.graph && (p.graph_B != B || p.graph_S_cap != p.S_cap || p.graph_Tar != Tar || p.graph_ws != workspace)) {
    STG(sopro_graph_destroy(p.graph));
    p.graph = nullptr;
  }
  return 0;
}

int sopro_ar_run_graph(sopro_engine* e, int32_t n_steps, void* stream) {
  SOPRO_CHECK_ARG(e && e->ar.ws && n_steps >= 0 && stream, "sopro_ar_begin first; a non-default stream is needed for graph capture");
  ArPlan& p = e->ar;
  if (!p.graph) {
    STG(sopro_capture_begin(stream));
    const int rc = ar_issue_step(e, (hipStream_t)stream);
    void* g = nullptr;
    const int rc2 = sopro_capture_end(stream, &g);
    if (rc != 0) return rc;
    if (rc2 != 0) return rc2;
    p.graph = g; p.graph_B = p.B; p.graph_S_cap = p.S_cap; p.graph_Tar = p.Tar; p.graph_ws = p.ws;
  }
  for (int i = 0; i < n_steps; ++i) STG(sopro_graph_launch(p.graph, stream));
  return 0;
}

int sopro_ar_tokens(sopro_engine* e, int32_t* hist, int32_t* first_eos, int32_t* n_stopped, void* stream) {
  SOPRO_CHECK_ARG(e && e->ar.ws, "sopro_ar_begin first");
  hipStream_t s = (hipStream_t)stream;
  const ArPlan& p = e->ar;
  if (hist) STG(sopro_copy2d_u32(hist, (int64_t)p.B * p.Tar, p.hist, (int64_t)p.B * p.Tar, 1, p.B * p.Tar, s));
  if (first_eos) STG(sopro_copy2d_u32(first_eos, p.B, p.first_eos, p.B, 1, p.B, s));
  if (n_stopped) STG(sopro_copy2d_u32(n_stopped, 1, p.ctr + 2, 1, 1, 1, s));
  return 0;
}

struct NarWs { float *xa, *xb, *h, *x1, *u, *z, *part, *cond; int32_t *lens, *range; SplitK sk; };
static size_t nar_carve(const sopro_engine* e, NarWs& w, void* ws, int B, int T) {
  const sopro_engine_cfg& c = e->c;
  const size_t M = (size_t)B * T, D = c.d_model;
  int nh_max = 0;
  for (int i = 0; i < c.n_stages; ++i) nh_max = c.stage_n_cb[i] > nh_max ? c.stage_n_cb[i] : nh_max;
  Carver cv(ws);
  w.xa = cv.take<float>(M * D); w.xb = cv.take<float>(M * D); w.h = cv.take<float>(M * D); w.x1 = cv.take<float>(M * D);
  w.u = cv.take<float>(M * 4 * D); w.z = cv.take<float>(M * c.nar_head_dim);
  w.part = cv.take<float>(M * nh_max * (c.codebook_size / 64) * 2);
  w.cond = cv.take<float>(M * D);
  w.lens = cv.take<int32_t>(B);
  w.range = cv.take<int32_t>(4);
  w.sk.tickets = cv.take<int32_t>(SPLITK_TICKETS);
  w.sk.ws = M <= 1024 ? cv.take<float>(SPLITK_WS_BYTES / 4) : nullptr;
  return cv.off;
}

int64_t sopro_nar_workspace_bytes(const sopro_engine* e, int32_t B, int32_t T) {
  if (!e || B <= 0 || T <= 0) return 0;
  NarWs w;
  return (int64_t)nar_carve(e, w, nullptr, B, T);
}

static int ssm_block_bufs(sopro_engine* e, hipStream_t s, float* h, float* x1, float* u, const SplitK* sk, const float* x, float* out,
                          const std::string& p, int B, int T, int ksize, int dil, const int32_t* lens, const char* sfx, int32_t* range) {
  const int D = e->c.d_model, M = B * T;
  const int total = (ksize - 1) * dil, left = total / 2;
  G g; g.M = M; g.N = 2 * D; g.K = D; g.bias = F(e, p + ".glu.b"); g.epi = SOPRO_EPI_GLU; g.rms_eps = RMS_EPS; g.range_events = range;
  STG(gemm(s, x, WT(e, p + ".glu.wn" + sfx), nullptr, h, g));
  STG(sopro_dwconv_f32(h, F(e, p + ".dw.w"), F(e, p + ".dw.b"), x, x1, lens, B, T, D, ksize, dil, left, 1, s));
  G f1; f1.M = M; f1.N = 4 * D; f1.K = D; f1.bias = F(e, p + ".ff1.b"); f1.epi = SOPRO_EPI_GELU; f1.rms_eps = RMS_EPS; f1.range_events = range;
  STG(gemm(s, x1, WT(e, p + ".ff1.wn" + sfx), nullptr, u, f1));
  G f2; f2.M = M; f2.N = D; f2.K = 4 * D; f2.bias = F(e, p + ".ff2.b"); f2.epi = SOPRO_EPI_RES; f2.R = x1; f2.sk = sk; f2.range_events = range;
  return gemm(s, u, WT(e, p + ".ff2.w" + sfx), nullptr, out, f2);
}
static int ssm_block_seq(sopro_engine* e, hipStream_t s, const NarWs& w, const float* x, float* out, const std::string& p, int B, int T,
                         int ksize, int dil, const int32_t* lens, const char* sfx) {
  return ssm_block_bufs(e, s, w.h, w.x1, w.u, &w.sk, x, out, p, B, T, ksize, dil, lens, sfx, w.range);
}

int sopro_nar_refine_io(sopro_engine* e, void* workspace, const sopro_nar_io* io, int32_t B, int32_t T, void* stream) {
  SOPRO_CHECK_ARG(e && e->final && e->has_nar && workspace && io && io->cond && io->cb0 && io->tokens && B > 0 && T > 0,
                  "bad arguments (finalize the engine with the NAR tensors first)");
  hipStream_t s = (hipStream_t)stream;
  const sopro_engine_cfg& c = e->c;
  const int D = c.d_model, V = c.codebook_size, Q = c.num_codebooks, HD = c.nar_head_dim, M = B * T;
  SOPRO_CHECK_ARG(V % 64 == 0, "codebook_size must be a multiple of 64 (arg-max partials per 64 columns)");
  SOPRO_CHECK_ARG(io->cond_bstride >= (int64_t)T * D && io->cb0_bstride >= T, "cond / cb0 blocks shorter than T rows");
  const bool safe = io->safe != 0 && c.precision == 0;
  const char* sfx = safe ? NAR_SAFE : "";
  int32_t* tokens = io->tokens;
  NarWs w;
  nar_carve(e, w, workspace, B, T);
  if (w.sk.ws) STG(sopro_fill2d_u32(w.sk.tickets, SPLITK_TICKETS, 1, SPLITK_TICKETS, 0u, s));
  STG(sopro_fill2d_u32(w.range, 4, 1, 4, 0u, s));
  int nh_max = 0;
  for (int i = 0; i < c.n_stages; ++i) nh_max = c.stage_n_cb[i] > nh_max ? c.stage_n_cb[i] : nh_max;
  const float* cnd = io->cond;
  if (io->cond_bstride != (int64_t)T * D) {
    STG(sopro_copy2d_u32(w.cond, (int64_t)T * D, io->cond, io->cond_bstride, B, T * D, s));
    cnd = w.cond;
  }
  STG(sopro_nar_seed_i32(tokens, Q, io->cb0, io->cb0_bstride, B, T, V - 1, s));
  const int32_t* lens_d = nullptr;
  if (io->lens) {
    STG(sopro_copy2d_u32(w.lens, B, io->lens, B, 1, B, s));
    lens_d = w.lens;
  }
  const char* stage_names[8] = {"B", "C", "D", "E", "F", "G", "H", "I"};
  for (int sid = 0; sid < c.n_stages; ++sid) {
    float *xa = w.xa, *xb = w.xb;
    STG(sopro_codebook_sum_f32(tokens, Q, e->nar_cols[sid], e->nar_offs[sid], e->nar_cw[sid], e->nar_known[sid], F(e, "cb_embed"),
                               e->t["cb_embed"].shape[0], cnd, c.nar_mix[sid][0], c.nar_mix[sid][1], xa, D, 0, M, M, D, s));
    STG(norm(s, xa, xb, F(e, "nar.adapter.norm.weight"), M, D, RMS_EPS, SOPRO_NORM_RMS, nullptr, e->ad_mul[sid], e->ad_add[sid], M));
    std::swap(xa, xb);
    for (int i = 0; i < c.n_layers_nar; ++i) {
      STG(ssm_block_seq(e, s, w, xa, xb, "nar.blocks." + std::to_string(i), B, T, c.nar_kernel, c.nar_dilations[i], lens_d, sfx));
      std::swap(xa, xb);
    }
    STG(norm(s, xa, xb, F(e, "nar.norm.weight"), M, D, RMS_EPS));
    G pz; pz.M = M; pz.N = HD; pz.K = D; pz.bias = F(e, "nar.pre.b"); pz.range_events = w.range;
    STG(gemm(s, xb, WT(e, std::string("nar.pre.w") + sfx), nullptr, w.z, pz));
    const int nh = c.stage_n_cb[sid];
    const std::string hk = std::string("nar.heads.") + stage_names[sid];
    G hg; hg.M = M; hg.N = nh * V; hg.K = HD; hg.bias = F(e, hk + ".b"); hg.c_mode = 5; hg.C2 = w.part; hg.ldc2 = (int64_t)nh_max * (V / 64);
    hg.range_events = w.range;
    STG(gemm(s, w.z, WT(e, hk + ".w" + sfx), nullptr, nullptr, hg));
    STG(sopro_argmax_partials_i32(w.part, (int64_t)nh_max * (V / 64), tokens + c.stage_first_cb[sid], Q, nh, V / 64, V, M, s));
  }
  if (io->range_out) STG(sopro_copy2d_u32(io->range_out, 1, w.range, 1, 1, 1, s));
  return 0;
}

int sopro_nar_refine(sopro_engine* e, void* workspace, const float* cond, int64_t cond_bstride, const int32_t* rvq1, const int32_t* lens,
                     int32_t B, int32_t T, int32_t* tokens, void* stream) {
  sopro_nar_io io;
  memset(&io, 0, sizeof(io));
  io.cond = cond; io.cond_bstride = cond_bstride; io.cb0 = rvq1; io.cb0_bstride = T; io.lens = lens; io.tokens = tokens;
  return sopro_nar_refine_io(e, workspace, &io, B, T, stream);
}

struct SeaLevel {
  int ch, co, rows, orow, r, hid;
  bool last;
  bool fused;
  bool res128;
};
struct MimiWs {
  int32_t* tok;
  float *emb, *q, *X, *y, *qkv, *ao, *hd, *e0, *hraw[8], *hact[8], *y1[8];
  float* lnst;
  SplitK sk;
  SeaLevel lv[8];
};
static bool mimi_half(const sopro_engine* e) {
  static const bool off = getenv("SOPRO_MIMI_BF16") != nullptr && getenv("SOPRO_MIMI_BF16")[0] == '0';
  return e->c.precision == 1 && !off;
}

static bool seanet_fused(int B, int rows) {
  static const bool off = SOPRO_DEV_ENV("SOPRO_SEANET_FUSE") != nullptr && SOPRO_DEV_ENV("SOPRO_SEANET_FUSE")[0] == '0';
  return !off && (int64_t)B * rows >= 512 * 1024;
}

static void sea_levels(const sopro_engine_cfg& c, int B, int T, SeaLevel* lv) {
  int ch = c.mimi_num_filters << c.mimi_n_ratios, rows = 2 * T;
  for (int si = 0; si < c.mimi_n_ratios; ++si) {
    SeaLevel& l = lv[si];
    l.ch = ch; l.co = ch / 2; l.rows = rows; l.r = c.mimi_ratios[si]; l.orow = rows * l.r; l.hid = l.co / c.mimi_compress;
    l.last = si + 1 == c.mimi_n_ratios;
    l.fused = l.last && ch == 128 && l.r == 4 && seanet_fused(B, rows);
    l.res128 = l.co == 128 && l.hid == 64;
    ch = l.co; rows = l.orow;
  }
}

enum ActFmt { ACT_F32 = 0, ACT_SPLIT = 1, ACT_BF16 = 2 };
enum ActOut { OUT_RAW = 0, OUT_ACT = 1, OUT_RAW_ACT = 2 };
static int act_c_mode(ActOut what, ActFmt f) {
  static const int mode[3][3] = {{0, 3, 4}, {0, 1, 2}, {6, 7, 8}};
  return mode[f][what];
}
static float* act_at(float* p, ActFmt f, size_t n) {
  return f == ACT_BF16 ? reinterpret_cast<float*>(reinterpret_cast<uint16_t*>(p) + n) : p + n;
}

static size_t mimi_carve(const sopro_engine* e, MimiWs& w, void* ws, int B, int T) {
  const sopro_engine_cfg& c = e->c;
  const bool half = mimi_half(e);
  auto act = [&](Carver& cv_, size_t n) { return half ? reinterpret_cast<float*>(cv_.take<uint16_t>(n)) : cv_.take<float>(n); };
  const size_t HS = c.mimi_hidden, CD = c.mimi_codebook_dim, N2 = 2 * (size_t)T, PADX = c.mimi_kernel - 1;
  Carver cv(ws);
  w.tok = cv.take<int32_t>((size_t)B * T * c.num_codebooks);
  w.sk.tickets = cv.take<int32_t>(SPLITK_TICKETS);
  w.sk.ws = (size_t)B * N2 <= 512 ? cv.take<float>(SPLITK_WS_BYTES / 4) : nullptr;
  w.emb = cv.take<float>((size_t)B * T * 2 * CD);
  w.q = cv.take<float>((size_t)B * T * HS);
  w.X = cv.take<float>((size_t)B * (PADX + N2) * HS);
  w.y = cv.take<float>((size_t)B * N2 * HS);
  w.qkv = cv.take<float>((size_t)B * N2 * 3 * HS);
  w.ao = cv.take<float>((size_t)B * N2 * HS);
  w.hd = cv.take<float>((size_t)B * N2 * c.mimi_inter);
  w.lnst = cv.take<float>((size_t)B * N2 * ((HS + 63) / 64) * 2);
  sea_levels(c, B, T, w.lv);
  w.e0 = act(cv, (size_t)B * (1 + N2) * ((size_t)c.mimi_num_filters << c.mimi_n_ratios));
  for (int si = 0; si < c.mimi_n_ratios; ++si) {
    const SeaLevel& l = w.lv[si];
    w.hraw[si] = l.fused ? nullptr : act(cv, (size_t)B * (2 + l.orow) * l.co);
    w.hact[si] = l.last ? nullptr : act(cv, (size_t)B * (2 + l.orow) * l.co);
    w.y1[si] = l.last ? nullptr : act(cv, (size_t)B * l.orow * l.hid);
// ... 438 lines not shown
```

sopro_amd/hip.py:

```python
from __future__ import annotations

import ctypes as C
import gc
import os
import struct
import threading
from typing import List, Optional, Tuple

import torch

_HERE = os.path.dirname(os.path.abspath(__file__))
LIB_PATH = os.path.join(_HERE, "libsopro_hip.so")
ABI_VERSION = 43
DEV_MODE = os.environ.get("SOPRO_DEV", "0") == "1"


def dev_env(name: str, default: str) -> str:
    return os.environ.get(name, default) if DEV_MODE else default


DEFAULT_GROUP_M = 8
PRO_NONE, PRO_ELU, PRO_ADDVEC = 0, 1, 2
EPI_ROPE = 6
EPI_NONE, EPI_GELU, EPI_GLU, EPI_RES, EPI_TANH, EPI_GLU_DW = 0, 1, 2, 3, 4, 5
# ... 68 lines not shown

class EngineCfg(C.Structure):
    _fields_ = [("d_model", _i32), ("codebook_size", _i32), ("num_codebooks", _i32), ("nar_head_dim", _i32), ("bos_row", _i32),
                ("n_layers_ar", _i32), ("ar_kernel", _i32), ("ar_dilations", _i32 * 16), ("ar_xattn", _i32 * 16), ("ar_gate", _f32 * 16),
                ("n_layers_nar", _i32), ("nar_kernel", _i32), ("nar_dilations", _i32 * 16),
                ("n_stages", _i32), ("stage_first_cb", _i32 * 8), ("stage_n_cb", _i32 * 8), ("nar_mix", (_f32 * 2) * 8),
                ("nar_prev_cb_weights", _f32 * 64),
                ("mimi_hidden", _i32), ("mimi_codebook_dim", _i32), ("mimi_heads", _i32), ("mimi_head_dim", _i32), ("mimi_layers", _i32),
                ("mimi_window", _i32), ("mimi_inter", _i32), ("mimi_n_ratios", _i32), ("mimi_ratios", _i32 * 8), ("mimi_num_filters", _i32),
                ("mimi_kernel", _i32), ("mimi_res_kernel", _i32), ("mimi_last_kernel", _i32), ("mimi_compress", _i32),
                ("mimi_n_semantic", _i32), ("mimi_rope_positions", _i32), ("mimi_norm_eps", _f32), ("mimi_final_bias", _f32), ("precision", _i32),
                ("n_layers_text", _i32), ("ref_enc_layers", _i32), ("ref_xattn_layers", _i32), ("ref_xattn_heads", _i32), ("sv_student_dim", _i32),
                ("enc_kernel", _i32)]


class NarIO(C.Structure):
    _fields_ = [("cond", _p), ("cond_bstride", _i64), ("cb0", _p), ("cb0_bstride", _i64), ("lens", _p), ("tokens", _p), ("range_out", _p),
                ("safe", _i32)]


class MimiStreamState(C.Structure):
    _fields_ = [("kv", _p), ("cap_rows", _i32), ("kv_len", _i32), ("pos", _i32), ("evict", _i32), ("half", _i32)]


class MimiStreamBatch(C.Structure):
    _fields_ = [("kv", _p), ("rows_cap", _i32), ("rows", _i32), ("cap_rows", _i32), ("kv_len", _i32), ("pos", _i32), ("evict", _i32),
                ("half", _i32)]


SYMBOLS = {
    "sopro_last_error": (C.c_char_p, []),
    "sopro_abi_version": (C.c_int, []),
    "sopro_build_flags": (C.c_int, []),
    "sopro_graph_launch_n": (C.c_int, [_p, _p, _i32]),
    "sopro_host_alloc": (C.c_int, [_i64, C.POINTER(_p)]),
    "sopro_host_free": (C.c_int, [_p]),
    "sopro_copy_to_host_async": (C.c_int, [_p, _p, _i64, _p]),
    "sopro_set_lds_floor": (C.c_int, [C.c_int]),
    "sopro_set_host_wait": (C.c_int, [C.c_int]),
    "sopro_device_info": (C.c_int, [C.c_int, C.POINTER(C.c_int)]),
    "sopro_capture_begin": (C.c_int, [_p]),
    "sopro_capture_end": (C.c_int, [_p, C.POINTER(_p)]),
    "sopro_graph_launch": (C.c_int, [_p, _p]),
    "sopro_graph_destroy": (C.c_int, [_p]),
    "sopro_stream_create_cu_range": (C.c_int, [C.c_int, C.c_int, C.POINTER(_p)]),
    "sopro_stream_create_cu_mask": (C.c_int, [_p, _i32, _p]),
    "sopro_stream_destroy": (C.c_int, [_p]),
    "sopro_gemm_f32": (C.c_int, [C.POINTER(GemmArgs), _p]),
    "sopro_gemm_bf16x3": (C.c_int, [_p, _p, _p, _p]),
    "sopro_gemm_bf16x6": (C.c_int, [_p, _p, _p, _p]),
    "sopro_gemm_bf16x1": (C.c_int, [_p, _p, _p, _p]),
    "sopro_pack_w_bf16": (C.c_int, [_p, _i64, _i32, _i32, _i32, _p, _p]),
    "sopro_fill2d_u32": (C.c_int, [_p, _i64, _i32, _i32, C.c_uint32, _p]),
    "sopro_copy2d_u32": (C.c_int, [_p, _i64, _p, _i64, _i32, _i32, _p]),
    "sopro_pack_w_f16x2": (C.c_int, [_p, _i64, _i32, _i32, _f32, _p, _p]),
    "sopro_f16x3_a_scale": (C.c_float, []),
    "sopro_gemm_f16x3": (C.c_int, [_p, _p, _p, _p]),
    "sopro_packed_w_bytes": (C.c_int64, [_i32, _i32, _i32]),
    "sopro_packed_w_rows_bytes": (C.c_int64, [_i32, _i32]),
    "sopro_pack_w_rows_bf16": (C.c_int, [_p, _i64, _i32, _i32, _p, _p]),
    "sopro_gemm_8p_takes": (C.c_int, [_p, _p]),
    "sopro_gemm_auto_ksplit": (C.c_int, [C.c_int32, C.c_int32, C.c_int32, C.c_int32, C.c_int32, C.c_int32, C.c_int64, C.c_int32]),
    "sopro_gemm_bf16x3_8p": (C.c_int, [_p, _p, _p, _p]),
    "sopro_gemm_bf16_set_tile_override": (C.c_int, [C.c_int]),
    "sopro_gemm_set_group_m": (C.c_int, [C.c_int]),
    "sopro_seanet_tail_set_tiles": (C.c_int, [C.c_int]),
    "sopro_seanet_res_set_tiles": (C.c_int, [C.c_int]),
    "sopro_seanet_res128_bf16": (C.c_int, [_p, _i64, _p, _p, _p, _p, _p, _i64, _i32, _i32, _p]),
    "sopro_seanet_up128_bf16": (C.c_int, [_p, _i64, _p, _p, _p, _i64, _i32, _i32, _p]),
    "sopro_seanet_tail_bf16": (C.c_int, [_p, _i64, _p, _p, _p, _p, _p, _f32, _p, _i64, _i32, _i32, _p]),
    "sopro_seanet_up_set_tiles": (C.c_int, [C.c_int]),
    "sopro_seanet_uptail_set_tiles": (C.c_int, [C.c_int]),
    "sopro_seanet_uptail_f32": (C.c_int, [_p, _i64, _p, _p, _p, _p, _p, _p, _p, _f32, _p, _i64, _i32, _i32, _i32, _p]),
    "sopro_seanet_uptail_bf16": (C.c_int, [_p, _i64, _p, _p, _p, _p, _p, _p, _p, _f32, _p, _i64, _i32, _i32, _p]),
    "sopro_seanet_up128_f32": (C.c_int, [_p, _i64, _p, _p, _p, _i64, _i32, _i32, _i32, _p]),
    "sopro_seanet_res128_f32": (C.c_int, [_p, _i64, _p, _p, _p, _p, _p, _i64, _i32, _i32, _p]),
    "sopro_gemm_set_tile_override": (C.c_int, [C.c_int]),
    "sopro_pack_skinny_w": (C.c_int, [_p, _i64, _i32, _i32, _i32, _p, _p]),
    "sopro_pack_skinny_w_bf16": (C.c_int, [_p, _i64, _i32, _i32, _i32, _p, _p]),
    "sopro_skinny_packed_floats": (_i64, [_i32, _i32, _i32]),
    "sopro_skinny_f32": (C.c_int, [C.POINTER(SkinnyArgs), _p]),
    "sopro_row_stats_f32": (C.c_int, [_p, _i64, _i64, _i32, _i32, _i32, _p, _p]),
    "sopro_norm_f32": (C.c_int, [_p, _i64, _i64, _p, _i64, _p, _p, _p, _p, _i32, _i32, _i32, _f32, _i32, _p]),
    "sopro_rms_match_f32": (C.c_int, [_p, _p, _p, _i32, _i32, _p]),
    "sopro_tanh_affine_f32": (C.c_int, [_p, _p, _f32, _f32, _i64, _p]),
    "sopro_add_pos_f32": (C.c_int, [_p, _p, _p, _i32, _i32, _i32, _i32, _p]),
    "sopro_masked_mean_f32": (C.c_int, [_p, _p, _p, _i32, _i32, _i32, _p]),
    "sopro_stats_pool_f32": (C.c_int, [_p, _p, _p, _p, _i32, _i32, _i32, _p]),
    "sopro_l2norm_f32": (C.c_int, [_p, _p, _i32, _i32, _f32, _p]),
    "sopro_dwconv_f32": (C.c_int, [_p, _p, _p, _p, _p, _p, _i32, _i32, _i32, _i32, _i32, _i32, _i32, _p]),
    "sopro_codebook_sum_f32": (C.c_int, [_p, _i32, _p, _p, _p, _i32, _p, _i64, _p, _f32, _f32, _p, _i64, _i64, _i32, _i32, _i32, _p]),
    "sopro_text_embed_f32": (C.c_int, [_p, _p, _p, _i64, _p, _p, _i32, _i32, _i32, _p]),
    "sopro_argmax_rows_f32": (C.c_int, [_p, _i64, _p, _i64, _i32, _i32, _i32, _p]),
    "sopro_argmax_partials_i32": (C.c_int, [_p, _i64, _p, _i64, _i32, _i32, _i32, _i32, _p]),
    "sopro_fir1_f32": (C.c_int, [_p, _i64, _i32, _p, _p, _p, _i64, _i64, _i32, _i32, _i32, _i32, _i32, _i32, _p]),
    "sopro_rvq_assign_f32": (C.c_int, [_p, _i64, _i32, _p, _p, _i64, _i32, _p, _i64, _i32, _p]),
    "sopro_attention_f32": (C.c_int, [C.POINTER(AttnArgs), _p]),
    "sopro_attention_split_bf16": (C.c_int, [C.POINTER(AttnArgs), C.c_int32, _p]),
    "sopro_attn_decode_f32": (C.c_int, [C.POINTER(AttnArgs), _p]),
    "sopro_xattn_step_f32": (C.c_int, [C.POINTER(XattnArgs), _p]),
    "sopro_rope_f32": (C.c_int, [_p, _i64, _p, _p, _i32, _i32, _i32, _i32, _i32, _p]),
    "sopro_upsample2_f32": (C.c_int, [_p, _p, _p, _i64, _i32, _i32, _i32, _p]),
    "sopro_final_conv_f32": (C.c_int, [_p, _i64, _p, _f32, _p, _i64, _i32, _i32, _p]),
    "sopro_seanet_tail_f32": (C.c_int, [_p, _i64, _p, _p, _p, _p, _p, _f32, _p, _i64, _i32, _i32, _p]),
    "sopro_seanet_res128_p_f32": (C.c_int, [_p, _i64, _p, _p, _p, _p, _p, _i64, _i32, _i32, _i32, _p]),
    "sopro_seanet_tail_p_f32": (C.c_int, [_p, _i64, _p, _p, _p, _p, _p, _f32, _p, _i64, _i32, _i32, _i32, _p]),
    "sopro_engine_create": (C.c_int, [C.POINTER(EngineCfg), C.POINTER(_p)]),
    "sopro_engine_set_tensor": (C.c_int, [_p, C.c_char_p, _p, C.POINTER(_i64), _i32]),
    "sopro_engine_finalize": (C.c_int, [_p, _p]),
    "sopro_engine_destroy": (C.c_int, [_p]),
    "sopro_ar_workspace_bytes": (_i64, [_p, _i32, _i32, _i32]),
    "sopro_ar_begin": (C.c_int, [_p, _p, _i32, _p, _p, _p, _i32, _i32, C.POINTER(_f32), C.c_uint64, C.c_uint32, _p]),
    "sopro_ar_run_graph": (C.c_int, [_p, _i32, _p]),
    "sopro_ar_tokens": (C.c_int, [_p, _p, _p, _p, _p]),
    "sopro_nar_workspace_bytes": (_i64, [_p, _i32, _i32]),
    "sopro_nar_refine": (C.c_int, [_p, _p, _p, _i64, _p, _p, _i32, _i32, _p, _p]),
    "sopro_nar_refine_io": (C.c_int, [_p, _p, C.POINTER(NarIO), _i32, _i32, _p]),
    "sopro_nar_seed_i32": (C.c_int, [_p, _i32, _p, _i64, _i32, _i32, _i32, _p]),
    "sopro_mimi_workspace_bytes": (_i64, [_p, _i32, _i32]),
    "sopro_mimi_decode": (C.c_int, [_p, _p, _p, _i32, _i32, _p, _p]),
    "sopro_mimi_chunk_rows": (_i32, [_i32, _i32]),
    "sopro_mimi_decode_parts": (C.c_int, [_p, _p, _p, _i32, _i32, _p, _i32, _p]),
    "sopro_mimi_stream_kv_bytes": (_i64, [_p, _i32]),
    "sopro_mimi_stream_init": (C.c_int, [_p, C.POINTER(MimiStreamState), _p, _i32]),
    "sopro_mimi_stream_trim": (C.c_int, [C.POINTER(MimiStreamState), _i32]),
    "sopro_mimi_decode_stream": (C.c_int, [_p, _p, C.POINTER(MimiStreamState), _p, _i32, _p, _p]),
    "sopro_mimi_stream_batch_kv_bytes": (_i64, [_p, _i32, _i32]),
    "sopro_mimi_stream_batch_init": (C.c_int, [_p, C.POINTER(MimiStreamBatch), _p, _i32, _i32]),
    "sopro_mimi_stream_batch_trim": (C.c_int, [C.POINTER(MimiStreamBatch), _i32]),
    "sopro_mimi_stream_batch_keep": (C.c_int, [_p, C.POINTER(MimiStreamBatch), C.POINTER(_i32), _i32, _p]),
    "sopro_mimi_decode_stream_batch": (C.c_int, [_p, _p, C.POINTER(MimiStreamBatch), _p, _i32, _p, _p]),
    "sopro_ar_init": (C.c_int, [C.POINTER(ArState), _p]),
    "sopro_ar_sample": (C.c_int, [C.POINTER(ArState), _p, _i64, _p]),
    "sopro_ar_admit": (C.c_int, [C.POINTER(ArState), _i32, _p]),
    "sopro_ar_issue_frame": (C.c_int, [C.POINTER(ArFrame), _p]),
    "sopro_ar_fold_text": (C.c_int, [_p, _p, _p, _p, _p, _p, _p, _p, _p, _i32, _i32, _i32, _i32, _i32, _f32, _p]),
    "sopro_ar_fold_text_uk": (C.c_int, [_p, _p, _p, _p, _p, _p, _p, _p, _i32, _i32, _i32, _i32, _i32, _f32, _p]),
    "sopro_engine_upload_tensor": (C.c_int, [_p, C.c_char_p, _p, C.POINTER(_i64), _i32, _p]),
    "sopro_checkpoint_open": (C.c_int, [C.c_char_p, C.c_char_p, C.POINTER(_p)]),
    "sopro_checkpoint_close": (C.c_int, [_p]),
    "sopro_checkpoint_count": (_i32, [_p]),
    "sopro_checkpoint_tensor": (C.c_int, [_p, _i32, C.POINTER(C.c_char_p), C.POINTER(_p), C.POINTER(_i64), C.POINTER(_i32)]),
    "sopro_checkpoint_engine_cfg": (C.c_int, [_p, _i32, C.POINTER(EngineCfg)]),
    "sopro_engine_from_checkpoint": (C.c_int, [_p, _i32, _p, C.POINTER(_p)]),
    "sopro_engine_set_ar_tiles": (C.c_int, [_p, _i32, _i32, _i32, _i32]),
    "sopro_cond_workspace_bytes": (_i64, [_p, _i32, _i32, _i32]),
    "sopro_cond_prepare": (C.c_int, [_p, _p, _p, _p, _i32, _p, _p, _p, _p, _i64, _p, _p, _i32, _i32, _i32, _i32, _p, _p, _p, _p]),
    "sopro_film_coeffs": (C.c_int, [_p, _p, _f32, _i32, _p, _p, _p, _p]),
    "sopro_ref_workspace_bytes": (_i64, [_p, _i32]),
    "sopro_ref_prepare": (C.c_int, [_p, _p, _p, _i32, _p, _p, _p, _p]),
    "sopro_mimi_encode_workspace_bytes": (_i64, [_p, _i32, _i32]),
    "sopro_mimi_encode": (C.c_int, [_p, _p, _p, _i32, _i32, _p, _p]),
    "sopro_cvt_f32_bf16": (C.c_int, [_p, _p, _i64, _p]),
    "sopro_cvt_bf16_f32": (C.c_int, [_p, _p, _i64, _p]),
    "sopro_prof_enable": (C.c_int, [C.c_int]),
    "sopro_prof_collect": (C.c_int, [_p, _i32, _p]),
    "sopro_join_workspace_bytes": (_i64, [_i32, _i64, _i32]),
    "sopro_join_edges_f32": (C.c_int, [_p, _i64, _p, _i32, _i64, _i32, _f32, _i32, _i32, _p, _p, _p]),
    "sopro_join_layout_i64": (C.c_int, [_p, _p, _i32, _p, _p]),
    "sopro_join_mix_f32": (C.c_int, [_p, _i64, _p, _p, _p, _i32, _i32, _p, _i64, _p]),
    "sopro_tsm_out_len": (_i64, [_i64, _i64]),
    "sopro_tsm_blocks": (_i64, [_i64]),
    "sopro_tsm_chunk_out_cap": (_i64, [_i64]),
    "sopro_tsm_state_bytes": (_i64, [_i32]),
    "sopro_tsm_rows_f32": (C.c_int, [_p, _i64, _p, _i64, _p, _i32, _p, _i32, _p, _p, _i64, _i64, _p, _p, _i32, _p]),
    "sopro_pitch_out_len": (_i64, [_i64, _i64]),
# ... 133 lines not shown
    if rc != 0:
        raise SoproHipError(f"{what} failed ({rc}): {load().sopro_last_error().decode()}")


def _stream() -> int:
    return torch.cuda.current_stream().cuda_stream


def ptr(t: Optional[torch.Tensor], dtype: torch.dtype = torch.float32) -> Optional[int]:
    if t is None:
        return None
    if not t.is_cuda:
        raise SoproHipError("tensor is not on a HIP device: the Sopro hot path has no CPU fallback")
    if t.dtype != dtype:
        raise SoproHipError(f"expected {dtype}, got {t.dtype}")
    return t.data_ptr()


def gemm(A: torch.Tensor, W, Cout: torch.Tensor, *, M: int, N: int, K: int, lda: Optional[int] = None,
         ldc: Optional[int] = None, bias: Optional[torch.Tensor] = None, epilogue: int = EPI_NONE,
         prologue: int = PRO_NONE, R: Optional[torch.Tensor] = None, ldr: Optional[int] = None,
         scale: Optional[torch.Tensor] = None, pro_vec: Optional[torch.Tensor] = None, rows_per_seg: Optional[int] = None,
         a_seg_stride: int = 0, c_seg_stride: int = 0, r_seg_stride: int = 0, a_off: int = 0, c_off: int = 0,
         r_off: int = 0, ldw: Optional[int] = None, dbg: Optional[torch.Tensor] = None, a_split: bool = False, c_mode: int = 0,
         C2: Optional[torch.Tensor] = None, ldc2: Optional[int] = None, c2_seg_stride: int = 0,
         c2_off: int = 0, rms_eps: float = 0.0, range_events: Optional[torch.Tensor] = None, rope: Optional[tuple] = None,
         ln_stats: Optional[torch.Tensor] = None, ln_eps: float = 0.0, ln_stats_out: Optional[torch.Tensor] = None,
         long_k: Optional[bool] = None, ksplit: Optional[int] = None, group_m: Optional[int] = None) -> None:
    n_out = N // 2 if epilogue == EPI_GLU else N
    g = GemmArgs()
    a16 = A.dtype == torch.bfloat16
    c16 = c_mode in (6, 7, 8)
    cdt = torch.bfloat16 if c16 else torch.float32
    g.A = ptr(A, A.dtype if a16 else torch.float32) + (2 if a16 else 4) * a_off
    g.lda = K if lda is None else lda
    g.a_seg_stride = a_seg_stride
    packed = isinstance(W, PackedW)
    if packed and (W.N != N or W.K != K):
        raise SoproHipError(f"packed weight is [{W.N}, {W.K}], the call wants [{N}, {K}]")
    g.W = None if packed else ptr(W)
    g.ldw = K if ldw is None else ldw
    g.bias = ptr(bias)
    g.C = (ptr(Cout, cdt) + (2 if c16 else 4) * c_off) if Cout is not None else None
    g.ldc = n_out if ldc is None else ldc
    g.c_seg_stride = c_seg_stride
    g.R = (ptr(R, cdt) + (2 if c16 else 4) * r_off) if R is not None else None
    g.ldr = (n_out if ldr is None else ldr)
    g.r_seg_stride = r_seg_stride
    g.scale = ptr(scale)
    g.pro_vec = ptr(pro_vec)
    g.dbg = ptr(dbg, torch.int64)
    g.M, g.N, g.K = M, N, K
    g.rows_per_seg = M if rows_per_seg is None else rows_per_seg
    g.prologue, g.epilogue = prologue, epilogue
    e0 = _prof.begin() if _prof is not None else None
    x = None
    if packed:
        x = SplitExt()
        if rope is not None:
            x.rope_cos, x.rope_sin = ptr(rope[0]), ptr(rope[1])
            x.rope_cols, x.rope_dh, x.rope_pos0, x.rope_rows_per_seg = int(rope[2]), int(rope[3]), int(rope[4]), int(rope[5])
        if ln_stats is not None:
            x.ln_stats, x.rms_eps = ptr(ln_stats), float(ln_eps)
        x.ln_stats_out = ptr(ln_stats_out)
        if rms_eps > 0.0:
            if W.pieces == 2 and not W.f16:
                raise SoproHipError("fused RMSNorm is a six-pass (pieces = 3), f16 three-pass or one-pass (pieces = 1) feature")
            x.rms_norm, x.rms_eps = 1, float(rms_eps)
        if group_m is not None:
            x.group_m = int(group_m)
        if ksplit is not None:
            ks = int(ksplit)
            t64 = -(-M // 64) * -(-N // 64)
            if ks > 1 and (ks * t64 * 64 * 64 * 4 > _SPLITK_WS_BYTES or t64 > _SPLITK_TICKETS):
                raise SoproHipError(f"ksplit={ks}: {M} x {N} does not fit the split-K workspace / tickets of a stream")
        else:
            ks = _auto_ksplit(M, N, K, W.pieces, epilogue, W.f16) if (dbg is None and _splitk_enabled and rms_eps <= 0.0) else 1
        if ks > 1 or ksplit is not None:
            ws, tk = _splitk_buffers()
            x.ksplit, x.n_tickets, x.ws, x.ws_bytes, x.tickets = ks, int(tk.numel()), ptr(ws), int(ws.numel()) * 4, ptr(tk, torch.int32)
    if (a16 or c16) and not (packed and W.pieces == 1 and not W.f16):
        raise SoproHipError("bf16 rows (a_format 2, c_mode 6 / 7 / 8) belong to the one-pass (pieces = 1) path")
    if packed and W.f16:
        if a_split or c_mode not in (0, 5):
            raise SoproHipError("split-form operands belong to the bf16 three-pass (pieces = 2) path")
        if c_mode == 5:
            x.c_mode, x.C2, x.ldc2 = 5, ptr(C2) + 4 * c2_off, (-(-N // 64) if ldc2 is None else ldc2)
        x.acc_scale = W.acc_scale
        x.range_events = ptr(range_events, torch.int32)
        _check(load().sopro_gemm_f16x3(C.byref(g), ptr(W.data, torch.int32), C.byref(x), _stream()), "sopro_gemm_f16x3")
    elif packed and W.pieces == 1:
        if a_split or c_mode in (1, 2):
            raise SoproHipError("split-form operands belong to the three-pass (pieces = 2) path")
        x.c_mode = c_mode
        x.a_format = 2 if a16 else 0
        x.C2 = (ptr(C2, cdt) + (2 if c16 else 4) * c2_off) if C2 is not None else None
        x.ldc2, x.c2_seg_stride = (n_out if ldc2 is None else ldc2), c2_seg_stride
        _check(load().sopro_gemm_bf16x1(C.byref(g), ptr(W.data, torch.int32), C.byref(x), _stream()), "sopro_gemm_bf16x1")
    elif packed and W.pieces == 3:
        if a_split or c_mode not in (0, 5):
            raise SoproHipError("split-form operands belong to the three-pass (pieces = 2) path")
        if c_mode == 5:
            x.c_mode, x.C2, x.ldc2 = 5, ptr(C2) + 4 * c2_off, (-(-N // 64) if ldc2 is None else ldc2)
        _check(load().sopro_gemm_bf16x6(C.byref(g), ptr(W.data, torch.int32), C.byref(x), _stream()), "sopro_gemm_bf16x6")
    elif packed:
        if a16 or c16:
            raise SoproHipError("bf16 rows (a_format 2, c_mode 6 / 7 / 8) belong to the one-pass (pieces = 1) path")
        x.a_format, x.c_mode = int(bool(a_split)), c_mode
        x.C2 = (ptr(C2) + 4 * c2_off) if C2 is not None else None
        x.ldc2, x.c2_seg_stride = (n_out if ldc2 is None else ldc2), c2_seg_stride
        use_8p = long_k if long_k is not None else (W.rows is not None and bool(load().sopro_gemm_8p_takes(C.byref(g), C.byref(x))))
        if use_8p:
            if W.rows is None:
                raise SoproHipError("the long-K form needs the weight's split-form rows (pack_w_bf16x3(W, rows=True))")
            x.ksplit = 0
            _check(load().sopro_gemm_bf16x3_8p(C.byref(g), W.rows.data_ptr(), C.byref(x), _stream()), "sopro_gemm_bf16x3_8p")
        else:
            _check(load().sopro_gemm_bf16x3(C.byref(g), ptr(W.data, torch.int32), C.byref(x), _stream()), "sopro_gemm_bf16x3")
    elif a_split or c_mode:
        raise SoproHipError("split-plane operands need a PackedW weight (the fp32 kernel reads and writes fp32 rows)")
    elif ksplit is not None or group_m is not None:
        raise SoproHipError("ksplit / group_m belong to the packed-weight paths (sopro_gemm_split_ext)")
    else:
        _check(load().sopro_gemm_f32(C.byref(g), _stream()), "sopro_gemm_f32")
    if e0 is not None:
        fam = "gemm_f32_kernel" if not packed else ("gemm_f16x3_kernel" if W.f16 else {1: "gemm_bf16x1_kernel", 2: "gemm_bf16x3_kernel", 3: "gemm_bf16x6_kernel"}[W.pieces])
        _prof.end(fam, 2.0 * M * N * K, e0)


_splitk_enabled = True
_splitk_pool: dict = {}
_SPLITK_WS_BYTES = 32 << 20
_SPLITK_TICKETS = 1024


def _auto_ksplit(M: int, N: int, K: int, pieces: int, epilogue: int, f16: bool = False) -> int:
    return load().sopro_gemm_auto_ksplit(M, N, K, pieces, int(f16), epilogue, _SPLITK_WS_BYTES, _SPLITK_TICKETS)


def _splitk_buffers():
    key = _stream()
    bufs = _splitk_pool.get(key)
    if bufs is None:
        dev = torch.cuda.current_device()
        bufs = (torch.empty(_SPLITK_WS_BYTES // 4, dtype=torch.float32, device=f"cuda:{dev}"),
                torch.zeros(_SPLITK_TICKETS, dtype=torch.int32, device=f"cuda:{dev}"))
        _splitk_pool[key] = bufs
    return bufs


class PackedW:

    __slots__ = ("data", "N", "K", "pieces", "f16", "acc_scale", "rows")

    def __init__(self, data: torch.Tensor, N: int, K: int, pieces: int, f16: bool = False, acc_scale: float = 1.0):
        self.data, self.N, self.K, self.pieces, self.f16, self.acc_scale = data, N, K, pieces, f16, acc_scale
        self.rows = None


def pack_w_bf16(W: torch.Tensor, pieces: int) -> PackedW:
    if W.dim() != 2 or not W.is_contiguous():
        raise SoproHipError("pack_w_bf16 wants a contiguous [N, K] matrix")
    N, K = int(W.shape[0]), int(W.shape[1])
    lib = load()
    data = torch.empty(int(lib.sopro_packed_w_bytes(N, K, pieces)) // 4, dtype=torch.int32, device=W.device)
    _check(lib.sopro_pack_w_bf16(ptr(W), K, N, K, pieces, ptr(data, torch.int32), _stream()), "sopro_pack_w_bf16")
    return PackedW(data, N, K, pieces)

# ... 22 lines not shown
    lib = load()
    amax = float(W.abs().max())
    wscale = 2.0 ** (13 - math.frexp(amax)[1] + 1) if amax > 0.0 else 1.0
    data = torch.empty(int(lib.sopro_packed_w_bytes(N, K, 2)) // 4, dtype=torch.int32, device=W.device)
    _check(lib.sopro_pack_w_f16x2(ptr(W), K, N, K, wscale, ptr(data, torch.int32), _stream()), "sopro_pack_w_f16x2")
    return PackedW(data, N, K, 2, f16=True, acc_scale=1.0 / (float(lib.sopro_f16x3_a_scale()) * wscale))


def pack_w_bf16x6(W: torch.Tensor) -> PackedW:
    return pack_w_bf16(W, 3)


def pack_w_bf16x1(W: torch.Tensor) -> PackedW:
    return pack_w_bf16(W, 1)


class SkinnyW:

    __slots__ = ("data", "N", "K", "glu", "bf16")

    def __init__(self, data: torch.Tensor, N: int, K: int, glu: bool, bf16: bool = False):
        self.data, self.N, self.K, self.glu, self.bf16 = data, N, K, glu, bf16


def pack_skinny_w(W: torch.Tensor, glu: bool = False, bf16: bool = False) -> SkinnyW:
    N, K = int(W.shape[0]), int(W.shape[1])
    n = int(load().sopro_skinny_packed_floats(N, K, int(glu)))
    if n <= 0:
        raise SoproHipError(f"pack_skinny_w: unsupported shape {N}x{K} (K % 32 == 0; glu: N even)")
    Wc = W.contiguous()
    with torch.cuda.device(W.device):
        if bf16:
            out = torch.empty(n // 2, dtype=torch.int32, device=W.device)
            _check(load().sopro_pack_skinny_w_bf16(ptr(Wc), K, N, K, int(glu), ptr(out, torch.int32), _stream()), "sopro_pack_skinny_w_bf16")
        else:
            out = torch.empty(n, dtype=torch.float32, device=W.device)
            _check(load().sopro_pack_skinny_w(ptr(Wc), K, N, K, int(glu), ptr(out), _stream()), "sopro_pack_skinny_w")
    return SkinnyW(out, N, K, bool(glu), bool(bf16))


def skinny(X: torch.Tensor, W, Y: torch.Tensor, *, B: int, N: int, K: int, ldx: Optional[int] = None,
           ldy: Optional[int] = None, rms_norm: bool = False, eps: float = 1e-6, bias: Optional[torch.Tensor] = None,
           epilogue: int = EPI_NONE, R: Optional[torch.Tensor] = None, ldr: Optional[int] = None,
           scale: Optional[torch.Tensor] = None, ring: Optional[torch.Tensor] = None, dw_w: Optional[torch.Tensor] = None,
           dw_b: Optional[torch.Tensor] = None, step: Optional[torch.Tensor] = None, ring_len: int = 0, ring_bcap: int = 0,
           dil: int = 1, ksize: int = 1, Xp: Optional[torch.Tensor] = None, np_: int = 0, xp_stride: int = 0,
           ksplit: bool = False, y_part_stride: int = 0, dbg: Optional[torch.Tensor] = None, mt: int = 1, nt: int = 1,
           aux_W=None, aux_Y: Optional[torch.Tensor] = None, aux_bias: Optional[torch.Tensor] = None, aux_R: Optional[torch.Tensor] = None,
           aux_flags: int = 0, aux_y_part_stride: int = 0) -> None:
    a = SkinnyArgs()
    a.X, a.ldx = ptr(X), (K if ldx is None else ldx)
    if isinstance(W, SkinnyW):
        if (W.N, W.K, W.glu) != (N, K, epilogue == EPI_GLU_DW):
            raise SoproHipError(f"packed weight is {W.N}x{W.K} glu={W.glu}, the call says {N}x{K} glu={epilogue == EPI_GLU_DW}")
        a.W, a.ldw, a.w_layout = (ptr(W.data, torch.int32), K, 2) if W.bf16 else (ptr(W.data), K, 1)
    else:
        a.W, a.ldw = ptr(W), K
    a.bias = ptr(bias)
    n_out = N // 2 if epilogue == EPI_GLU_DW else N
    a.Y, a.ldy = ptr(Y), (n_out if ldy is None else ldy)
    a.R, a.ldr, a.scale = ptr(R), (n_out if ldr is None else ldr), ptr(scale)
    ring_bf16 = ring is not None and ring.dtype == torch.bfloat16
    a.ring, a.dw_w, a.dw_b, a.step = ptr(ring, torch.bfloat16 if ring_bf16 else torch.float32), ptr(dw_w), ptr(dw_b), ptr(step, torch.int32)
    a.ring_format = 1 if ring_bf16 else 0
    a.Xp, a.xp_stride, a.y_part_stride, a.dbg = ptr(Xp), xp_stride, y_part_stride, ptr(dbg, torch.int64)
    a.eps = eps
    a.B, a.N, a.K, a.epilogue = B, N, K, epilogue
    a.ring_len, a.ring_bcap, a.dil, a.ksize = ring_len, ring_bcap, dil, ksize
    a.np, a.ksplit, a.rms_norm = np_, int(ksplit), int(rms_norm)
    a.mt, a.nt = int(mt), int(nt)
    if aux_W is not None:
        if not isinstance(aux_W, SkinnyW) or aux_W.K != K or aux_W.glu or aux_W.bf16 != (a.w_layout == 2):
            raise SoproHipError("aux_W must be a packed (non-GLU) weight of the same K and element type as W")
        a.aux_W = ptr(aux_W.data, torch.int32) if aux_W.bf16 else ptr(aux_W.data)
        a.aux_tiles, a.aux_flags = (aux_W.N + 15) // 16, int(aux_flags)
        a.aux_Y, a.aux_ldy, a.aux_bias, a.aux_R, a.aux_ldr = ptr(aux_Y), aux_W.N, ptr(aux_bias), ptr(aux_R), aux_W.N
        a.aux_y_part_stride = aux_y_part_stride
    _check(load().sopro_skinny_f32(C.byref(a), _stream()), "sopro_skinny_f32")


def norm(x: torch.Tensor, out: torch.Tensor, w: torch.Tensor, *, rows: int, C_: int, eps: float, kind: int = NORM_RMS,
         b: Optional[torch.Tensor] = None, mul: Optional[torch.Tensor] = None, add: Optional[torch.Tensor] = None,
         rows_per_seg: Optional[int] = None, ldx: Optional[int] = None, ldo: Optional[int] = None, x_off: int = 0,
         o_off: int = 0, x_seg_stride: int = 0) -> None:
    _check(load().sopro_norm_f32(ptr(x) + 4 * x_off, C_ if ldx is None else ldx, x_seg_stride, ptr(out) + 4 * o_off,
                                 C_ if ldo is None else ldo, ptr(w), ptr(b), ptr(mul), ptr(add), rows,
                                 rows if rows_per_seg is None else rows_per_seg, C_, eps, kind, _stream()), "sopro_norm_f32")


def row_stats(x: torch.Tensor, rows: int, C_: int, stats: torch.Tensor, ldx: Optional[int] = None, x_seg_stride: int = 0,
              rows_per_seg: Optional[int] = None, x_off: int = 0) -> None:
    _check(load().sopro_row_stats_f32(ptr(x) + 4 * x_off, C_ if ldx is None else ldx, x_seg_stride, rows, rows if rows_per_seg is None else rows_per_seg,
                                      C_, ptr(stats), _stream()), "sopro_row_stats_f32")


def rms_match(a: torch.Tensor, x: torch.Tensor, out: torch.Tensor, rows: int, C_: int) -> None:
    _check(load().sopro_rms_match_f32(ptr(a), ptr(x), ptr(out), rows, C_, _stream()), "sopro_rms_match_f32")


def tanh_affine(x: torch.Tensor, out: torch.Tensor, c0: float, c1: float, n: int) -> None:
    _check(load().sopro_tanh_affine_f32(ptr(x), ptr(out), c0, c1, n, _stream()), "sopro_tanh_affine_f32")


def add_pos(rowvec: torch.Tensor, table: torch.Tensor, out: torch.Tensor, B: int, T: int, C_: int, pos0: int = 0) -> None:
    _check(load().sopro_add_pos_f32(ptr(rowvec), ptr(table), ptr(out), B, T, C_, pos0, _stream()), "sopro_add_pos_f32")


def masked_mean(x: torch.Tensor, lens: Optional[torch.Tensor], out: torch.Tensor, B: int, T: int, C_: int) -> None:
    _check(load().sopro_masked_mean_f32(ptr(x), ptr(lens, torch.int32), ptr(out), B, T, C_, _stream()), "sopro_masked_mean_f32")


def stats_pool(h: torch.Tensor, logit: torch.Tensor, lens: Optional[torch.Tensor], out: torch.Tensor, B: int, T: int, C_: int) -> None:
    _check(load().sopro_stats_pool_f32(ptr(h), ptr(logit), ptr(lens, torch.int32), ptr(out), B, T, C_, _stream()), "sopro_stats_pool_f32")


def l2norm(x: torch.Tensor, out: torch.Tensor, rows: int, C_: int, eps: float = 1e-6) -> None:
    _check(load().sopro_l2norm_f32(ptr(x), ptr(out), rows, C_, eps, _stream()), "sopro_l2norm_f32")


def dwconv(x: torch.Tensor, w: torch.Tensor, bias: Optional[torch.Tensor], out: torch.Tensor, *, B: int, T: int, C_: int,
           ksize: int, dil: int, left: int, mode: int = 0, res: Optional[torch.Tensor] = None,
           lens: Optional[torch.Tensor] = None) -> None:
    _check(load().sopro_dwconv_f32(ptr(x), ptr(w), ptr(bias), ptr(res), ptr(out), ptr(lens, torch.int32), B, T, C_, ksize,
                                   dil, left, mode, _stream()), "sopro_dwconv_f32")


def codebook_sum(tok: torch.Tensor, ldt: int, col: torch.Tensor, off: torch.Tensor, wq: torch.Tensor, table: torch.Tensor,
                 out: torch.Tensor, *, rows: int, D: int, base: Optional[torch.Tensor] = None, alpha: float = 0.0,
                 beta: float = 1.0, ldo: Optional[int] = None, rows_per_seg: Optional[int] = None, o_seg_stride: int = 0,
                 o_off: int = 0, tok_off: int = 0) -> None:
    _check(load().sopro_codebook_sum_f32(ptr(tok, torch.int32) + 4 * tok_off, ldt, ptr(col, torch.int32), ptr(off, torch.int32),
                                         ptr(wq), int(col.numel()), ptr(table), int(table.shape[0]), ptr(base), alpha, beta,
                                         ptr(out) + 4 * o_off, D if ldo is None else ldo, o_seg_stride, rows,
                                         rows if rows_per_seg is None else rows_per_seg, D, _stream()), "sopro_codebook_sum_f32")


def text_embed(ids: torch.Tensor, lens: Optional[torch.Tensor], table: torch.Tensor, pe: torch.Tensor, out: torch.Tensor,
               B: int, T: int, C_: int) -> None:
    _check(load().sopro_text_embed_f32(ptr(ids, torch.int32), ptr(lens, torch.int32), ptr(table), int(table.shape[0]), ptr(pe),
                                       ptr(out), B, T, C_, _stream()), "sopro_text_embed_f32")


def argmax_rows(x: torch.Tensor, out: torch.Tensor, *, rows: int, N: int, ldx: Optional[int] = None, ldo: int = 1,
                o_off: int = 0, inner: int = 1) -> None:
    _check(load().sopro_argmax_rows_f32(ptr(x), N if ldx is None else ldx, ptr(out, torch.int32) + 4 * o_off, ldo, inner, rows, N,
                                        _stream()), "sopro_argmax_rows_f32")


def argmax_partials(part: torch.Tensor, out: torch.Tensor, *, rows: int, heads: int, per_head: int, V: int, ldp: int, ldo: int = 1,
                    o_off: int = 0) -> None:
    _check(load().sopro_argmax_partials_i32(ptr(part), ldp, ptr(out, torch.int32) + 4 * o_off, ldo, heads, per_head, V, rows, _stream()),
           "sopro_argmax_partials_i32")


def fir1(x: torch.Tensor, w: torch.Tensor, out: torch.Tensor, *, B: int, n_in: int, n_out: int, C_: int, K: int, stride: int,
         left: int, bias: Optional[torch.Tensor] = None, ldo: Optional[int] = None, x_seg_stride: Optional[int] = None,
         o_seg_stride: Optional[int] = None, o_off: int = 0) -> None:
    ldo = C_ if ldo is None else ldo
    _check(load().sopro_fir1_f32(ptr(x), n_in if x_seg_stride is None else x_seg_stride, n_in, ptr(w), ptr(bias) if bias is not None else None,
                                 ptr(out) + 4 * o_off, ldo, n_out * ldo if o_seg_stride is None else o_seg_stride, B, n_out, C_, K,
                                 stride, left, _stream()), "sopro_fir1_f32")


def rvq_assign(scores: torch.Tensor, table: torch.Tensor, res: torch.Tensor, codes: torch.Tensor, *, rows: int, V: int, D: int,
               ldc: int, t_off: int = 0, c_off: int = 0) -> None:
    _check(load().sopro_rvq_assign_f32(ptr(scores), V, V, ptr(table) + 4 * t_off, ptr(res), D, D, ptr(codes, torch.int32) + 4 * c_off,
                                       ldc, rows, _stream()), "sopro_rvq_assign_f32")
# ... 1462 lines not shown
```

Measured before the change: 27810 audio-s/s.

## Pass NAR intermediates between f16x3 GEMMs in pre-split f16 hi/lo form

The FF1 GEMM in each NAR SSM block now writes its output as split f16 hi/lo pairs (c_mode 9), and FF2 reads that form directly (a_format 1). The same applies to the final norm, pre-projection and head GEMM chain, using a new split16 RMSNorm kernel. This removes the per-GEMM fp32-to-f16 split work in the A-operand prologue and keeps activation traffic the same size, while moving range-overflow counting into the producer. It adds new template instantiations and alignment constraints, and it is on by default but can be turned off through an environment variable.

```diff
diff --git a/include/sopro_hip.h b/include/sopro_hip.h
--- a/include/sopro_hip.h
+++ b/include/sopro_hip.h
@@ -120,6 +120,9 @@
 int sopro_norm_f32(const float* x, int64_t ldx, int64_t x_seg_stride , float* out, int64_t ldo, const float* w, const float* b,
                    const float* mul, const float* add, int32_t rows, int32_t rows_per_seg, int32_t C,
                    float eps, int32_t kind, void* stream);
+int sopro_norm_split16_f32(const float* x, int64_t ldx, int64_t x_seg_stride , void* out, int64_t ldo, const float* w, const float* b,
+                           const float* mul, const float* add, int32_t rows, int32_t rows_per_seg, int32_t C,
+                           float eps, int32_t kind, int32_t* range_events, void* stream);
 int sopro_row_stats_f32(const float* x, int64_t ldx, int64_t x_seg_stride , int32_t rows, int32_t rows_per_seg, int32_t C,
                         float* stats, void* stream);
 int sopro_rms_match_f32(const float* a, const float* x, float* out, int32_t rows, int32_t C, void* stream);
diff --git a/sopro_amd/csrc/common.h b/sopro_amd/csrc/common.h
--- a/sopro_amd/csrc/common.h
+++ b/sopro_amd/csrc/common.h
@@ -86,6 +86,20 @@
   lo = *reinterpret_cast<const unsigned*>(&l);
 }
 
+constexpr float SOPRO_A16_SCALE = 8.0f;
+constexpr float SOPRO_F16_MAX = 65504.0f;
+typedef _Float16 f16x2_t __attribute__((ext_vector_type(2)));
+__device__ __forceinline__ void split2_f16(float x, float y, unsigned& hi, unsigned& lo, bool& bad) {
+  const float vx = x * SOPRO_A16_SCALE, vy = y * SOPRO_A16_SCALE;
+  bad = bad || !(fabsf(vx) <= SOPRO_F16_MAX) || !(fabsf(vy) <= SOPRO_F16_MAX);
+  const f32x2_t v = {__builtin_amdgcn_fmed3f(vx, -SOPRO_F16_MAX, SOPRO_F16_MAX), __builtin_amdgcn_fmed3f(vy, -SOPRO_F16_MAX, SOPRO_F16_MAX)};
+  const f16x2_t h = __builtin_convertvector(v, f16x2_t);
+  hi = *reinterpret_cast<const unsigned*>(&h);
+  const f32x2_t r = {v[0] - (float)h[0], v[1] - (float)h[1]};
+  const f16x2_t l = __builtin_convertvector(r, f16x2_t);
+  lo = *reinterpret_cast<const unsigned*>(&l);
+}
+
 #ifndef SOPRO_NT_BULK
 #define SOPRO_NT_BULK 1
 #endif
diff --git a/sopro_amd/csrc/elementwise.hip b/sopro_amd/csrc/elementwise.hip
--- a/sopro_amd/csrc/elementwise.hip
+++ b/sopro_amd/csrc/elementwise.hip
@@ -4,10 +4,11 @@
 
 constexpr int NORM_MAX_PER_LANE = 16;
 
+template <bool SPLIT16>
 __global__ __launch_bounds__(256) void norm_kernel(const float* __restrict__ x, int64_t ldx, int64_t x_seg_stride, float* __restrict__ out,
                                                    int64_t ldo, const float* __restrict__ w, const float* __restrict__ b,
                                                    const float* __restrict__ mul, const float* __restrict__ add, int rows,
-                                                   int rows_per_seg, int C, float eps, int kind) {
+                                                   int rows_per_seg, int C, float eps, int kind, int32_t* __restrict__ range_events) {
   const int lane = threadIdx.x & 63;
   const int row = blockIdx.x * 4 + (threadIdx.x >> 6);
   if (row >= rows) return;
@@ -43,6 +44,7 @@
   const float* mr = mul ? mul + (int64_t)seg * C : nullptr;
   const float* ar = add ? add + (int64_t)seg * C : nullptr;
   float* orow = out + (int64_t)row * ldo;
+  bool bad = false;
 #pragma unroll
   for (int j = 0; j < NORM_MAX_PER_LANE; ++j) {
     const int c = lane + j * 64;
@@ -51,8 +53,19 @@
       if (b) y += b[c];
       if (mr) y *= mr[c];
       if (ar) y += ar[c];
-      orow[c] = y;
+      if constexpr (SPLIT16) {
+        unsigned hi, lo;
+        split2_f16(y, 0.f, hi, lo, bad);
+        unsigned short* g = reinterpret_cast<unsigned short*>(orow + (c & ~31)) + (c & 31);
+        g[0] = (unsigned short)hi;
+        g[32] = (unsigned short)lo;
+      } else {
+        orow[c] = y;
+      }
     }
+  }
+  if constexpr (SPLIT16) {
+    if (range_events && __any(bad) && lane == 0) atomicAdd(range_events, 1);
   }
 }
 
@@ -530,8 +543,23 @@
   SOPRO_CHECK_ARG(x && out && w, "x, out, w must be non-NULL");
   SOPRO_CHECK_ARG(rows > 0 && C > 0 && C <= 64 * NORM_MAX_PER_LANE && rows_per_seg > 0, "rows > 0, 0 < C <= 1024");
   SOPRO_CHECK_ARG(kind == SOPRO_NORM_RMS || kind == SOPRO_NORM_LN, "unknown norm kind");
-  hipLaunchKernelGGL(norm_kernel, dim3(nblk(rows, 4)), dim3(256), 0, (hipStream_t)stream, x, ldx,
-                     x_seg_stride ? x_seg_stride : (int64_t)rows_per_seg * ldx, out, ldo, w, b, mul, add, rows, rows_per_seg, C, eps, kind);
+  hipLaunchKernelGGL(norm_kernel<false>, dim3(nblk(rows, 4)), dim3(256), 0, (hipStream_t)stream, x, ldx,
+                     x_seg_stride ? x_seg_stride : (int64_t)rows_per_seg * ldx, out, ldo, w, b, mul, add, rows, rows_per_seg, C, eps, kind,
+                     (int32_t*)nullptr);
+  SOPRO_LAUNCH_CHECK();
+}
+
+int sopro_norm_split16_f32(const float* x, int64_t ldx, int64_t x_seg_stride, void* out, int64_t ldo, const float* w, const float* b,
+                           const float* mul, const float* add, int32_t rows, int32_t rows_per_seg, int32_t C, float eps,
+                           int32_t kind, int32_t* range_events, void* stream) {
+  SOPRO_CHECK_ARG(x && out && w, "x, out, w must be non-NULL");
+  SOPRO_CHECK_ARG(rows > 0 && C > 0 && C <= 64 * NORM_MAX_PER_LANE && rows_per_seg > 0, "rows > 0, 0 < C <= 1024");
+  SOPRO_CHECK_ARG(kind == SOPRO_NORM_RMS || kind == SOPRO_NORM_LN, "unknown norm kind");
+  SOPRO_CHECK_ARG((C & 31) == 0 && (ldo & 31) == 0 && ldo >= C && (reinterpret_cast<uintptr_t>(out) & 127u) == 0,
+                  "split-form output rows must start on 128-byte boundaries (C, ldo multiples of 32)");
+  hipLaunchKernelGGL(norm_kernel<true>, dim3(nblk(rows, 4)), dim3(256), 0, (hipStream_t)stream, x, ldx,
+                     x_seg_stride ? x_seg_stride : (int64_t)rows_per_seg * ldx, reinterpret_cast<float*>(out), ldo, w, b, mul, add, rows,
+                     rows_per_seg, C, eps, kind, range_events);
   SOPRO_LAUNCH_CHECK();
 }
 
diff --git a/sopro_amd/csrc/gemm_bf16s.hip b/sopro_amd/csrc/gemm_bf16s.hip
--- a/sopro_amd/csrc/gemm_bf16s.hip
+++ b/sopro_amd/csrc/gemm_bf16s.hip
@@ -9,12 +9,11 @@
 
 typedef __bf16 bf16x8 __attribute__((ext_vector_type(8)));
 typedef _Float16 f16x8 __attribute__((ext_vector_type(8)));
-typedef _Float16 f16x2_t __attribute__((ext_vector_type(2)));
 
 __device__ __forceinline__ bf16x8 as_frag(const uint4& v) { return *reinterpret_cast<const bf16x8*>(&v); }
 __device__ __forceinline__ f16x8 as_frag16(const uint4& v) { return *reinterpret_cast<const f16x8*>(&v); }
 
-constexpr float A16_SCALE = 8.0f;
+constexpr float A16_SCALE = SOPRO_A16_SCALE;
 
 template <int NPL, bool F16 = false>
 __device__ __forceinline__ void split_pair(float x, float y, unsigned (&pc)[NPL]) {
@@ -69,6 +68,7 @@
   if (dbg && tid == 0) dbg[0] = clock64();
 
   static_assert(AMODE != 5 || NPL == 1, "bf16 rows are a one-pass (bf16 mode) operand form");
+  static_assert(AMODE != 2 || NPL == 2, "split-form rows hold two pieces");
   constexpr int AES = AMODE == 5 ? 2 : 4;
   const char* ap[A_F4];
 #pragma unroll
@@ -138,7 +138,7 @@
   auto lstore_piece = [&](int buf, float4 (&ra)[A_F4], const float4& pv, int i, bool fresh, bool first) {
     if constexpr (FOLD) {
       if constexpr (AMODE == 4) asm volatile("" : "+v"(rsc[i]), "+v"(ssq[i]));
-      else asm volatile("" : "+v"(sapin[i]));
+      else if constexpr (AMODE != 2) asm volatile("" : "+v"(sapin[i]));
     }
     if constexpr (AMODE == 5) {
       unsigned char* a = As + buf * BM * AROW + lrow * AROW + lc4 * 8;
@@ -346,6 +346,9 @@
     }
   }
   if (dbg && tid == 0) dbg[2] = clock64();
+  if constexpr (F16 && AMODE != 2) {
+    if (ext.range_events && !(a16max <= 65504.0f)) atomicAdd(ext.range_events, 1);
+  }
   if constexpr (SK) {
     constexpr int PER_THREAD = TM * TN * 16;
     const int tile = bid, ntile = gridDim.x;
@@ -402,7 +405,6 @@
   float cscale = 1.0f;
   if constexpr (F16) {
     cscale = AMODE == 4 ? ext.acc_scale * A16_SCALE : ext.acc_scale;
-    if (ext.range_events && !(a16max <= 65504.0f)) atomicAdd(ext.range_events, 1);
   }
   const float* rs = nullptr;
   if constexpr (AMODE == 4) {
@@ -534,7 +536,19 @@
 
 template <int NPL, int WM, int WN, int TM, int TN, bool F16 = false>
 int launch_cfg6(const sopro_gemm_args& g, const uint4* wp, int ksubs, const sopro_gemm_split_ext& ext, hipStream_t s) {
-  const int key = g.epilogue * 10 + amode_of(g, ext);
+  const int key = g.epilogue * 10 + amode_of(g, ext) + ext.c_mode * 1000;
+  if constexpr (F16) {
+#define SOPRO_CASE16(E, A, O) \
+  case (E) * 10 + (A) + (O) * 1000: return launch_one<NPL, WM, WN, TM, TN, ((E) == SOPRO_EPI_GELU ? SOPRO_EPI_GELU_FAST : (E)), A, O, true>(g, wp, ksubs, ext, s)
+    switch (key) {
+      SOPRO_CASE16(SOPRO_EPI_GELU, 4, 9);
+      SOPRO_CASE16(SOPRO_EPI_RES, 2, 0);
+      SOPRO_CASE16(SOPRO_EPI_NONE, 2, 9);
+      SOPRO_CASE16(SOPRO_EPI_NONE, 0, 9);
+      default: break;
+    }
+#undef SOPRO_CASE16
+  }
 #define SOPRO_CASE(E, A) \
   case (E) * 10 + (A): return launch_one<NPL, WM, WN, TM, TN, (((E) == SOPRO_EPI_GELU && (F16 || NPL != 3)) ? SOPRO_EPI_GELU_FAST : (E)), A, 0, F16>(g, wp, ksubs, ext, s)
   switch (key) {
@@ -614,7 +628,11 @@
 #define SOPRO_TILE(T, WM, WN, TM, TN)                                                                                                     \
   case T:                                                                                                                                 \
     if constexpr (!has_tile<NPL, F16, FORM>(T)) break;                                                                                    \
-    else if constexpr (FORM == FORM_ARGMAX) return launch_one<NPL, WM, WN, TM, TN, SOPRO_EPI_NONE, 0, 5, F16>(c.g, c.wp, c.ksubs, c.ext, c.s); \
+    else if constexpr (FORM == FORM_ARGMAX) {                                                                                             \
+      if constexpr (F16)                                                                                                                  \
+        if (c.ext.a_format == 1) return launch_one<NPL, WM, WN, TM, TN, SOPRO_EPI_NONE, 2, 5, F16>(c.g, c.wp, c.ksubs, c.ext, c.s);       \
+      return launch_one<NPL, WM, WN, TM, TN, SOPRO_EPI_NONE, 0, 5, F16>(c.g, c.wp, c.ksubs, c.ext, c.s);                                  \
+    }                                                                                                                                     \
     else if constexpr (FORM == FORM_CFG6) return launch_cfg6<NPL, WM, WN, TM, TN, F16>(c.g, c.wp, c.ksubs, c.ext, c.s);                  \
     else return launch_cfg3<NPL, WM, WN, TM, TN>(c.g, c.wp, c.ksubs, c.ext, c.s);
     SOPRO_TILES(SOPRO_TILE)
@@ -628,7 +646,7 @@
 int launch_argmax(const Call& c) {
   const sopro_gemm_args& g = c.g;
   const sopro_gemm_split_ext& ext = c.ext;
-  SOPRO_CHECK_ARG(g.epilogue == SOPRO_EPI_NONE && g.prologue == SOPRO_PRO_NONE && !ext.rms_norm && ext.a_format == 0,
+  SOPRO_CHECK_ARG(g.epilogue == SOPRO_EPI_NONE && g.prologue == SOPRO_PRO_NONE && !ext.rms_norm && (ext.a_format == 0 || (F16 && ext.a_format == 1)),
                   "arg-max output takes a plain contraction (no prologue / epilogue / fused norm)");
   SOPRO_CHECK_ARG(ext.C2 && ext.ldc2 >= (g.N + 63) / 64, "arg-max output: C2 = [M][ldc2 >= ceil(N / 64)] (value, index) pairs");
   static const bool tm1 = SOPRO_DEV_ENV("SOPRO_ARGMAX_TM") != nullptr && SOPRO_DEV_ENV("SOPRO_ARGMAX_TM")[0] == '1';
@@ -715,9 +733,24 @@
 template <bool F16>
 int forms_x6(const char* who, const sopro_gemm_args& g, const sopro_gemm_split_ext& ext) {
   if (F16) SOPRO_CHECK_AS(who, ext.acc_scale > 0.f, "acc_scale = 1 / (sopro_f16x3_a_scale() * the weight's pack scale) must be set");
-  SOPRO_CHECK_AS(who, ext.a_format == 0 && (ext.c_mode == 0 || ext.c_mode == 5),
+  const bool split_in = F16 && ext.a_format == 1, split_out = F16 && ext.c_mode == 9;
+  SOPRO_CHECK_AS(who, (ext.a_format == 0 || split_in) && (ext.c_mode == 0 || ext.c_mode == 5 || split_out),
                  F16 ? "the f16 three-pass path reads fp32 rows and writes fp32 rows, or arg-max partials (c_mode 5)"
                      : "the six-pass path reads fp32 rows and writes fp32 rows, or arg-max partials (c_mode 5)");
+  if (split_in) {
+    SOPRO_CHECK_AS(who, !ext.rms_norm, "split-f16 rows (a_format 1) feed plain forms: the fused-RMSNorm forms sum the squares of fp32 rows");
+    SOPRO_CHECK_AS(who, g.prologue == SOPRO_PRO_NONE && (g.epilogue == SOPRO_EPI_RES || g.epilogue == SOPRO_EPI_NONE),
+                   "split-f16 rows (a_format 1): no prologue, epilogue RES or NONE");
+    SOPRO_CHECK_AS(who, g.epilogue != SOPRO_EPI_NONE || ext.c_mode != 0, "split-f16 rows (a_format 1) with epilogue NONE: c_mode 5 or 9");
+    SOPRO_CHECK_AS(who, (g.K & 31) == 0 && (g.lda & 31) == 0 && (g.a_seg_stride & 31) == 0 && (reinterpret_cast<uintptr_t>(g.A) & 127u) == 0,
+                   "split-form A: K, lda, a_seg_stride multiples of 32 and a 128-byte aligned base");
+  }
+  if (split_out) {
+    SOPRO_CHECK_AS(who, (g.epilogue == SOPRO_EPI_GELU && ext.rms_norm) || (g.epilogue == SOPRO_EPI_NONE && !ext.rms_norm && g.prologue == SOPRO_PRO_NONE),
+                   "split-f16 output (c_mode 9): the fused-RMSNorm GELU form, or a plain projection (no prologue, epilogue NONE)");
+    SOPRO_CHECK_AS(who, (g.N & 31) == 0 && g.C && (reinterpret_cast<uintptr_t>(g.C) & 127u) == 0 && (g.ldc & 31) == 0 && (g.c_seg_stride & 31) == 0 && g.ldc >= g.N,
+                   "split-form output rows must start on 128-byte boundaries (N, ld, seg stride multiples of 32)");
+  }
   return check_rms(who, g, ext, false);
 }
 
diff --git a/sopro_amd/csrc/gemm_epilogue.h b/sopro_amd/csrc/gemm_epilogue.h
--- a/sopro_amd/csrc/gemm_epilogue.h
+++ b/sopro_amd/csrc/gemm_epilogue.h
@@ -14,7 +14,7 @@
   const int tid = threadIdx.x, lane = tid & 63, wave = tid >> 6;
   const int wm = wave / WN, wn = wave % WN;
   const int rps = g.rows_per_seg;
-  const bool big = (int64_t)g.M * g.N * (OUT >= 6 ? 2 : 4) >= SOPRO_BIG_BYTES;
+  const bool big = (int64_t)g.M * g.N * (OUT >= 6 && OUT <= 8 ? 2 : 4) >= SOPRO_BIG_BYTES;
   constexpr int CLD = BN + 4;
   constexpr bool RES_AHEAD = EPI == SOPRO_EPI_RES && OUT < 5;
   constexpr int RA_TPR = BN / 4, RA_RPP = NT / RA_TPR, RA_NPASS = BM / RA_RPP;
@@ -103,7 +103,7 @@
     }
     return;
   }
-  if constexpr (OUT >= 6) {
+  if constexpr (OUT >= 6 && OUT <= 8) {
     constexpr bool hres = EPI == SOPRO_EPI_RES;
     static_assert(EPI == SOPRO_EPI_NONE || EPI == SOPRO_EPI_RES, "bf16 rows take EPI_NONE or EPI_RES");
     constexpr int HTPR = BN / 4, HRPP = NT / HTPR, HNPASS = BM / HRPP;
@@ -224,7 +224,12 @@
   int seg = m / rps, rr = m - seg * rps;
   float* cptr = g.C + (int64_t)seg * g.c_seg_stride + (int64_t)rr * g.ldc + ocol;
   constexpr bool second = OUT == 2 || OUT == 4;
-  constexpr bool split_out = OUT == 1 || OUT == 2;
+  constexpr bool split_out = OUT == 1 || OUT == 2 || OUT == 9;
+  bool bad16 = false;
+  auto count16 = [&]() {
+    if constexpr (OUT == 9)
+      if (bad16 && ext->range_events) atomicAdd(ext->range_events, 1);
+  };
   float* const dbase = second ? ext->C2 : g.C;
   const int64_t ldd = second ? ext->ldc2 : g.ldc, dseg = second ? ext->c2_seg_stride : g.c_seg_stride;
   const int64_t dcol_bytes = split_out ? (int64_t)(ocol >> 5) * 128 + (ocol & 31) * 2 : (int64_t)ocol * 4;
@@ -272,7 +277,14 @@
           else { v.x = v.x * c4.x + pv.x * s4.x; v.y = v.y * c4.y + pv.y * s4.y; v.z = v.z * c4.z + pv.z * s4.z; v.w = v.w * c4.w + pv.w * s4.w; }
         }
       }
-      if (split_out) {
+      if constexpr (OUT == 9) {
+        uint2 h, l;
+        split2_f16(v.x, v.y, h.x, l.x, bad16);
+        split2_f16(v.z, v.w, h.y, l.y, bad16);
+        *reinterpret_cast<uint2*>(dpq) = h;
+        *reinterpret_cast<uint2*>(dpq + 64) = l;
+        return;
+      } else if (split_out) {
         uint2 h, l;
         split2_bf16(eluf_(v.x), eluf_(v.y), h.x, l.x);
         split2_bf16(eluf_(v.z), eluf_(v.w), h.y, l.y);
@@ -303,6 +315,7 @@
 #endif
       }
     }
+    count16();
     return;
   }
   auto batch = [&](int p0, const float4* rvb) {
@@ -346,4 +359,5 @@
 #endif
     }
   }
+  count16();
 }
diff --git a/sopro_amd/csrc/stages.hip b/sopro_amd/csrc/stages.hip
--- a/sopro_amd/csrc/stages.hip
+++ b/sopro_amd/csrc/stages.hip
@@ -1005,6 +1005,11 @@
   return (int64_t)nar_carve(e, w, nullptr, B, T);
 }
 
+static bool nar_split_on() {
+  const char* v = getenv("SOPRO_NAR_SPLIT");
+  return !(v && v[0] == '0');
+}
+
 static int ssm_block_bufs(sopro_engine* e, hipStream_t s, float* h, float* x1, float* u, const SplitK* sk, const float* x, float* out,
                           const std::string& p, int B, int T, int ksize, int dil, const int32_t* lens, const char* sfx, int32_t* range) {
   const int D = e->c.d_model, M = B * T;
@@ -1013,9 +1018,14 @@
   STG(gemm(s, x, WT(e, p + ".glu.wn" + sfx), nullptr, h, g));
   STG(sopro_dwconv_f32(h, F(e, p + ".dw.w"), F(e, p + ".dw.b"), x, x1, lens, B, T, D, ksize, dil, left, 1, s));
   G f1; f1.M = M; f1.N = 4 * D; f1.K = D; f1.bias = F(e, p + ".ff1.b"); f1.epi = SOPRO_EPI_GELU; f1.rms_eps = RMS_EPS; f1.range_events = range;
-  STG(gemm(s, x1, WT(e, p + ".ff1.wn" + sfx), nullptr, u, f1));
   G f2; f2.M = M; f2.N = D; f2.K = 4 * D; f2.bias = F(e, p + ".ff2.b"); f2.epi = SOPRO_EPI_RES; f2.R = x1; f2.sk = sk; f2.range_events = range;
-  return gemm(s, u, WT(e, p + ".ff2.w" + sfx), nullptr, out, f2);
+  const Wt &w1 = WT(e, p + ".ff1.wn" + sfx), &w2 = WT(e, p + ".ff2.w" + sfx);
+  if (w1.packed && w1.f16 && w2.packed && w2.f16 && (4 * D) % 32 == 0 && nar_split_on()) {
+    f1.c_mode = 9;
+    f2.a_fmt = 1;
+  }
+  STG(gemm(s, x1, w1, nullptr, u, f1));
+  return gemm(s, u, w2, nullptr, out, f2);
 }
 static int ssm_block_seq(sopro_engine* e, hipStream_t s, const NarWs& w, const float* x, float* out, const std::string& p, int B, int T,
                          int ksize, int dil, const int32_t* lens, const char* sfx) {
@@ -1061,14 +1071,19 @@
       STG(ssm_block_seq(e, s, w, xa, xb, "nar.blocks." + std::to_string(i), B, T, c.nar_kernel, c.nar_dilations[i], lens_d, sfx));
       std::swap(xa, xb);
     }
-    STG(norm(s, xa, xb, F(e, "nar.norm.weight"), M, D, RMS_EPS));
-    G pz; pz.M = M; pz.N = HD; pz.K = D; pz.bias = F(e, "nar.pre.b"); pz.range_events = w.range;
-    STG(gemm(s, xb, WT(e, std::string("nar.pre.w") + sfx), nullptr, w.z, pz));
     const int nh = c.stage_n_cb[sid];
     const std::string hk = std::string("nar.heads.") + stage_names[sid];
+    const Wt &wpre = WT(e, std::string("nar.pre.w") + sfx), &whd = WT(e, hk + ".w" + sfx);
+    const bool hsplit = wpre.packed && wpre.f16 && whd.packed && whd.f16 && D % 32 == 0 && HD % 32 == 0 && nar_split_on();
+    if (hsplit) STG(sopro_norm_split16_f32(xa, D, 0, xb, D, F(e, "nar.norm.weight"), nullptr, nullptr, nullptr, M, M, D, RMS_EPS, SOPRO_NORM_RMS, w.range, s));
+    else STG(norm(s, xa, xb, F(e, "nar.norm.weight"), M, D, RMS_EPS));
+    G pz; pz.M = M; pz.N = HD; pz.K = D; pz.bias = F(e, "nar.pre.b"); pz.range_events = w.range;
+    if (hsplit) { pz.a_fmt = 1; pz.c_mode = 9; }
+    STG(gemm(s, xb, wpre, nullptr, w.z, pz));
     G hg; hg.M = M; hg.N = nh * V; hg.K = HD; hg.bias = F(e, hk + ".b"); hg.c_mode = 5; hg.C2 = w.part; hg.ldc2 = (int64_t)nh_max * (V / 64);
     hg.range_events = w.range;
-    STG(gemm(s, w.z, WT(e, hk + ".w" + sfx), nullptr, nullptr, hg));
+    if (hsplit) hg.a_fmt = 1;
+    STG(gemm(s, w.z, whd, nullptr, nullptr, hg));
     STG(sopro_argmax_partials_i32(w.part, (int64_t)nh_max * (V / 64), tokens + c.stage_first_cb[sid], Q, nh, V / 64, V, M, s));
   }
   if (io->range_out) STG(sopro_copy2d_u32(io->range_out, 1, w.range, 1, 1, 1, s));
diff --git a/sopro_amd/hip.py b/sopro_amd/hip.py
--- a/sopro_amd/hip.py
+++ b/sopro_amd/hip.py
@@ -174,6 +174,7 @@
     "sopro_skinny_f32": (C.c_int, [C.POINTER(SkinnyArgs), _p]),
     "sopro_row_stats_f32": (C.c_int, [_p, _i64, _i64, _i32, _i32, _i32, _p, _p]),
     "sopro_norm_f32": (C.c_int, [_p, _i64, _i64, _p, _i64, _p, _p, _p, _p, _i32, _i32, _i32, _f32, _i32, _p]),
+    "sopro_norm_split16_f32": (C.c_int, [_p, _i64, _i64, _p, _i64, _p, _p, _p, _p, _i32, _i32, _i32, _f32, _i32, _p, _p]),
     "sopro_rms_match_f32": (C.c_int, [_p, _p, _p, _i32, _i32, _p]),
     "sopro_tanh_affine_f32": (C.c_int, [_p, _p, _f32, _f32, _i64, _p]),
     "sopro_add_pos_f32": (C.c_int, [_p, _p, _p, _i32, _i32, _i32, _i32, _p]),
@@ -473,8 +474,9 @@
     if (a16 or c16) and not (packed and W.pieces == 1 and not W.f16):
         raise SoproHipError("bf16 rows (a_format 2, c_mode 6 / 7 / 8) belong to the one-pass (pieces = 1) path")
     if packed and W.f16:
-        if a_split or c_mode not in (0, 5):
-            raise SoproHipError("split-form operands belong to the bf16 three-pass (pieces = 2) path")
+        if c_mode not in (0, 5, 9):
+            raise SoproHipError("split-bf16 outputs belong to the bf16 three-pass (pieces = 2) path")
+        x.a_format, x.c_mode = int(bool(a_split)), c_mode
         if c_mode == 5:
             x.c_mode, x.C2, x.ldc2 = 5, ptr(C2) + 4 * c2_off, (-(-N // 64) if ldc2 is None else ldc2)
         x.acc_scale = W.acc_scale
@@ -663,7 +665,13 @@
 def norm(x: torch.Tensor, out: torch.Tensor, w: torch.Tensor, *, rows: int, C_: int, eps: float, kind: int = NORM_RMS,
          b: Optional[torch.Tensor] = None, mul: Optional[torch.Tensor] = None, add: Optional[torch.Tensor] = None,
          rows_per_seg: Optional[int] = None, ldx: Optional[int] = None, ldo: Optional[int] = None, x_off: int = 0,
-         o_off: int = 0, x_seg_stride: int = 0) -> None:
+         o_off: int = 0, x_seg_stride: int = 0, split16: bool = False, range_events: Optional[torch.Tensor] = None) -> None:
+    if split16:
+        _check(load().sopro_norm_split16_f32(ptr(x) + 4 * x_off, C_ if ldx is None else ldx, x_seg_stride, ptr(out) + 4 * o_off,
+                                             C_ if ldo is None else ldo, ptr(w), ptr(b), ptr(mul), ptr(add), rows,
+                                             rows if rows_per_seg is None else rows_per_seg, C_, eps, kind,
+                                             ptr(range_events, torch.int32), _stream()), "sopro_norm_split16_f32")
+        return
     _check(load().sopro_norm_f32(ptr(x) + 4 * x_off, C_ if ldx is None else ldx, x_seg_stride, ptr(out) + 4 * o_off,
                                  C_ if ldo is None else ldo, ptr(w), ptr(b), ptr(mul), ptr(add), rows,
                                  rows if rows_per_seg is None else rows_per_seg, C_, eps, kind, _stream()), "sopro_norm_f32")
```

New measurement: 27690 audio-s/s. No clear change (-0.4%).
